# USCbiostats/bayesnetworks

Measured on NVIDIA B200. Metric: edge_proposals_scored_per_sec, higher is better.
Workload: dtype f64

## Files before the change

bayesnetworks_b200/api.py:

```python
from __future__ import annotations

import ctypes as C
from dataclasses import dataclass
from typing import Optional, Sequence

import numpy as np

from . import _lib
from ._lib import BN_RNG_REPLAY, BN_RNG_RMT, BN_RNG_WH, BnError, as_i32, check, ptr
from .network import Network

TRACE_COLUMNS = ("iter", "ChangedNode", "movetype", "globalLL", "additions", "deletions", "FN", "FP")
_RNG_KINDS = {"wh": BN_RNG_WH, "rmt": BN_RNG_RMT, "replay": BN_RNG_REPLAY,
              BN_RNG_WH: BN_RNG_WH, BN_RNG_RMT: BN_RNG_RMT, BN_RNG_REPLAY: BN_RNG_REPLAY}


@dataclass
class ChainResult:
    trace: dict
    uniforms: int
    valid_iters: int
    proposed: tuple
    reject: tuple
    n_nonpd: int
    total_edges: int
    windows: int
    alg_bytes: int
    phase_cycles: tuple
    slots_simulated: int
    final_parents: np.ndarray
    final_npar: np.ndarray
    accepted_moves: Optional[np.ndarray] = None
    edge_freq: Optional[np.ndarray] = None
    npar_freq: Optional[np.ndarray] = None
    kernel_cycles: int = 0
    mt_state: Optional[np.ndarray] = None
    state: Optional["ChainState"] = None

    def edges(self):
        return [(int(self.final_parents[c, e]), c)
                for c in range(len(self.final_npar)) for e in range(int(self.final_npar[c]))]


_STATE_SCALARS = ("iter", "valid", "total_edges_member", "additions", "deletions", "uniforms")


@dataclass
class ChainState:
    parents: np.ndarray
    npar: np.ndarray
    n_samples: Optional[int] = None
    rng: Optional[int] = None
    iter: int = 0
    valid: int = 1
    total_edges_member: int = 0
    additions: int = 0
    deletions: int = 0
    uniforms: int = 0
    wh_state: Optional[np.ndarray] = None
    mt_state: Optional[np.ndarray] = None
    score_block: Optional[np.ndarray] = None

    @property
    def P(self) -> int:
        return int(self.npar.shape[0])

    @property
    def max_par(self) -> int:
        return int(self.parents.shape[1])

    @property
    def resumed(self) -> bool:
        return self.rng is not None

    @classmethod
    def from_graph(cls, parents, npar) -> "ChainState":
        parents, npar = as_i32(parents), as_i32(npar)
        if parents.ndim != 2 or npar.shape != (parents.shape[0],):
            raise ValueError("parents must be (P, max_par) and npar (P,)")
        return cls(parents=parents.copy(), npar=npar.copy())

    @classmethod
    def from_edges(cls, edges, n_nodes: int, max_par: int) -> "ChainState":
        parents = np.full((n_nodes, max_par), -1, dtype=np.int32)
        npar = np.zeros(n_nodes, dtype=np.int32)
        for j, c in edges:
            if npar[c] >= max_par:
                raise ValueError(f"node {c} has more than max_par = {max_par} parents")
            parents[c, npar[c]] = j
            npar[c] += 1
        return cls(parents=parents, npar=npar)

    def save(self, path) -> None:
        d = {"parents": self.parents, "npar": self.npar}
        for k in _STATE_SCALARS:
            d[k] = np.int64(getattr(self, k))
        for k in ("n_samples", "rng"):
            if getattr(self, k) is not None:
                d[k] = np.int64(getattr(self, k))
        for k in ("wh_state", "mt_state", "score_block"):
            if getattr(self, k) is not None:
                d[k] = getattr(self, k)
        np.savez(path, **d)

    @classmethod
    def load(cls, path) -> "ChainState":
        with np.load(path) as z:
            kw = {k: int(z[k]) for k in _STATE_SCALARS}
            for k in ("n_samples", "rng"):
                kw[k] = int(z[k]) if k in z else None
            for k in ("wh_state", "mt_state", "score_block"):
                kw[k] = z[k].copy() if k in z else None
            return cls(parents=z["parents"].copy(), npar=z["npar"].copy(), **kw)


def _bad_arg(msg):
    return BnError(_lib.BN_ERR_BAD_ARG, msg)


def _i32_bits(a) -> np.ndarray:
    return np.ascontiguousarray((np.asarray(a).astype(np.int64) & 0xFFFFFFFF).astype(np.uint32).view(np.int32))


def set_default_stream(cuda_stream: Optional[int]) -> None:
    check(_lib.lib().bn_set_default_stream(C.c_void_p(cuda_stream or 0)))


class Context:

    def __init__(self, handle, n_samples, n_nodes, max_par):
        self._h = handle
        self.n_samples, self.n_nodes, self.max_par = n_samples, n_nodes, max_par

    @staticmethod
    def _graph_args(graph_source, graph_target, graph_node_type, n_nodes):
        src, tgt = as_i32(graph_source), as_i32(graph_target)
        if src.shape != tgt.shape:
            raise ValueError("graph_source and graph_target must have the same length")
        nt = as_i32(graph_node_type)
        if nt.shape != (n_nodes,):
            raise ValueError("graph_node_type must have one entry per column of X")
        return src, tgt, nt

    @classmethod
    def from_data(cls, X, graph_source, graph_target, graph_node_type, max_par=50, phi=1.0,
                  omega=6.9, device=0):
        Xf = np.asfortranarray(np.asarray(X, dtype=np.float64))
        n, p = Xf.shape
        src, tgt, nt = cls._graph_args(graph_source, graph_target, graph_node_type, p)
        h = C.c_void_p()
        check(_lib.lib().bn_create(ptr(Xf), n, p, ptr(src), ptr(tgt), len(src), ptr(nt), int(max_par),
                                   float(phi), float(omega), int(device), C.byref(h)))
        return cls(h, n, p, int(max_par))

    @classmethod
    def from_device(cls, data_ptr, ld, n_samples, n_nodes, graph_source, graph_target,
                    graph_node_type, max_par=50, phi=1.0, omega=6.9, device=0):
        src, tgt, nt = cls._graph_args(graph_source, graph_target, graph_node_type, n_nodes)
        h = C.c_void_p()
        check(_lib.lib().bn_create_from_device(C.c_void_p(int(data_ptr)), int(ld), int(n_samples),
                                               int(n_nodes), ptr(src), ptr(tgt), len(src), ptr(nt),
                                               int(max_par), float(phi), float(omega), int(device),
                                               C.byref(h)))
        return cls(h, int(n_samples), int(n_nodes), int(max_par))

    @classmethod
    def from_stats(cls, n_samples, mean, centered_gram, graph_source, graph_target,
                   graph_node_type, max_par=50, phi=1.0, omega=6.9, device=0):
        mean = np.ascontiguousarray(mean, dtype=np.float64)
        cg = np.ascontiguousarray(centered_gram, dtype=np.float64)
        p = mean.shape[0]
        if cg.shape != (p, p):
            raise ValueError("centered_gram must be (n_nodes, n_nodes)")
        src, tgt, nt = cls._graph_args(graph_source, graph_target, graph_node_type, p)
        h = C.c_void_p()
        check(_lib.lib().bn_create_from_stats(int(n_samples), p, ptr(mean), ptr(cg), ptr(src), ptr(tgt),
                                              len(src), ptr(nt), int(max_par), float(phi),
                                              float(omega), int(device), C.byref(h)))
        return cls(h, int(n_samples), p, int(max_par))

    @classmethod
    def from_stats_device(cls, n_samples, n_nodes, d_mean, d_centered_gram, graph_source, graph_target,
                          graph_node_type, max_par=50, phi=1.0, omega=6.9, device=0):
        src, tgt, nt = cls._graph_args(graph_source, graph_target, graph_node_type, n_nodes)
        h = C.c_void_p()
        check(_lib.lib().bn_create_from_stats_device(int(n_samples), int(n_nodes), C.c_void_p(int(d_mean)),
                                                     C.c_void_p(int(d_centered_gram)), ptr(src), ptr(tgt),
                                                     len(src), ptr(nt), int(max_par), float(phi), float(omega),
                                                     int(device), C.byref(h)))
        return cls(h, int(n_samples), int(n_nodes), int(max_par))

    def close(self):
        if self._h is not None and self._h.value:
            _lib.lib().bn_destroy(self._h)
            self._h = None

    def __enter__(self):
        return self

    def __exit__(self, *exc):
        self.close()

    def __del__(self):
        try:
            self.close()
        except Exception:
            pass

    def set_stream(self, cuda_stream: Optional[int]):
        check(_lib.lib().bn_set_stream(self._h, C.c_void_p(cuda_stream or 0)))

    @property
    def gram_ms(self) -> float:
        ms = C.c_float(0)
        check(_lib.lib().bn_get_gram_ms(self._h, C.byref(ms)))
        return float(ms.value)

    @property
    def launch_count(self) -> int:
        return int(_lib.lib().bn_get_launch_count(self._h))

    def stats(self):
        p = self.n_nodes
        sum_x, mean = np.empty(p), np.empty(p)
        sum_xx = np.empty((p, p), order="F")
        centered = np.empty((p, p))
        check(_lib.lib().bn_get_stats(self._h, ptr(sum_x), ptr(sum_xx), ptr(mean), ptr(centered)))
        return sum_x, np.ascontiguousarray(sum_xx), mean, centered

    def score_nodes(self, child, parents, n_par):
        child, n_par = as_i32(child), as_i32(n_par)
        parents = as_i32(parents)
        n = child.shape[0]
        if parents.shape != (n, self.max_par):
            raise ValueError(f"parents must be ({n}, {self.max_par})")
        out = np.empty(n)
        check(_lib.lib().bn_score_nodes(self._h, n, ptr(child), ptr(parents), ptr(n_par), ptr(out)))
        return out

    def score_all_proposals(self, parents, n_par, want_score=True, want_log_hr=True):
        parents, n_par = as_i32(parents), as_i32(n_par)
        if parents.ndim == 2:
            parents, n_par = parents[None], n_par[None]
        g, p = n_par.shape
        if parents.shape != (g, p, self.max_par) or p != self.n_nodes:
            raise ValueError("parents must be (n_graphs, n_nodes, max_par)")
        base = np.empty((g, p))
        score = np.empty((g, p, p)) if want_score else None
        hr = np.empty((g, p, p)) if want_log_hr else None
        check(_lib.lib().bn_score_all_proposals(self._h, g, ptr(parents), ptr(n_par), ptr(base),
                                                ptr(score), ptr(hr)))
        return base, score, hr

    def score_all_proposals_device(self, n_graphs, d_parents, d_npar, d_base, d_score, d_log_hr):
        ms = C.c_float(0)
        check(_lib.lib().bn_score_all_proposals_device(
            self._h, int(n_graphs), C.c_void_p(d_parents), C.c_void_p(d_npar), C.c_void_p(d_base or 0),
            C.c_void_p(d_score or 0), C.c_void_p(d_log_hr or 0), C.byref(ms)))
        return float(ms.value)

    @property
    def score_state_len(self) -> int:
        n = C.c_int64(0)
        check(_lib.lib().bn_score_state_len(self._h, C.byref(n)))
        return int(n.value)

    def _start_args(self, start, n_chains, kind, args, keep):
        p, mp = self.n_nodes, self.max_par
        if len(start) != n_chains:
            raise _bad_arg(f"start holds {len(start)} states for {n_chains} chains")
        for c, st in enumerate(start):
            if st.P != p or st.max_par != mp:
                raise _bad_arg(f"start state of chain {c} is for P={st.P}, max_par={st.max_par}; "
                               f"the context has P={p}, max_par={mp}")
            if st.resumed and (st.rng != kind or st.n_samples != self.n_samples):
                raise _bad_arg(f"start state of chain {c} continues a stream of kind {st.rng} over "
                               f"{st.n_samples} samples; this run is kind {kind} over {self.n_samples}")
        resumed = {st.resumed for st in start}
        if len(resumed) > 1:
            raise _bad_arg("start mixes fresh and resumed chains")
        par = np.ascontiguousarray(np.stack([as_i32(st.parents) for st in start]))
        npar = np.ascontiguousarray(np.stack([as_i32(st.npar) for st in start]))
        keep += [par, npar]
        args.start_parents, args.start_n_par = par.ctypes.data_as(_lib._ip), npar.ctypes.data_as(_lib._ip)
        if resumed.pop():
            sts = (_lib.ChainStateC * n_chains)()
            for c, st in enumerate(start):
                o = sts[c]
                for k in _STATE_SCALARS:
                    setattr(o, k, int(getattr(st, k)))
                if kind == BN_RNG_WH:
                    o.wh_state[:] = [int(v) for v in st.wh_state]
            keep.append(sts)
            args.state_in = C.cast(sts, C.c_void_p)
            if kind == BN_RNG_RMT:
                mt_in = np.ascontiguousarray(np.stack([_i32_bits(st.mt_state) for st in start]))
                keep.append(mt_in)
                args.mt_state_in = mt_in.ctypes.data_as(_lib._ip)
        blocks = [st.score_block is not None for st in start]
        if any(blocks):
            if not all(blocks):
                raise _bad_arg("start gives a score block for some chains only")
            sb = np.ascontiguousarray(np.stack([np.asarray(st.score_block, dtype=np.float64) for st in start]))
            if sb.shape[1] != self.score_state_len:
                raise _bad_arg(f"score block of {sb.shape[1]} doubles; this context needs {self.score_state_len}")
            keep.append(sb)
            args.score_state_in = sb.ctypes.data_as(_lib._dp)

    def run(self, n_chains=1, n_iter=1000, output=100, initial_network=2, drop=0, rng="wh",
            seeds=None, replay=None, log_moves=False, moves_capacity=None, tabulate=False,
            mt_state=None, want_mt_state=False, start=None, want_state=False):
        L = _lib.lib()
        kind = _RNG_KINDS[rng]
        p, mp = self.n_nodes, self.max_par
        cap = max(1, (n_iter + output - 1) // output)
        ints = {k: np.empty((n_chains, cap), dtype=np.int32) for k in
                ("iter", "ChangedNode", "movetype", "additions", "deletions", "FN", "FP")}
        gll = np.empty((n_chains, cap))
        n_rows = np.zeros(n_chains, dtype=np.int32)
        tr = _lib.Trace(cap, n_rows.ctypes.data_as(_lib._ip), ints["iter"].ctypes.data_as(_lib._ip),
                        ints["ChangedNode"].ctypes.data_as(_lib._ip),
                        ints["movetype"].ctypes.data_as(_lib._ip), gll.ctypes.data_as(_lib._dp),
                        ints["additions"].ctypes.data_as(_lib._ip),
                        ints["deletions"].ctypes.data_as(_lib._ip), ints["FN"].ctypes.data_as(_lib._ip),
                        ints["FP"].ctypes.data_as(_lib._ip))
        args = _lib.RunArgs()
        args.n_chains, args.rng_kind = int(n_chains), int(kind)
        sd = None
        if seeds is not None:
            sd = np.zeros((n_chains, 3), dtype=np.int32)
            s_in = np.asarray(seeds, dtype=np.int64)
            if s_in.ndim == 0:
                s_in = s_in.reshape(1, 1)
            if s_in.ndim == 1:
                s_in = s_in.reshape(n_chains, -1) if n_chains > 1 else s_in.reshape(1, -1)
            sd[:, :s_in.shape[1]] = s_in
            args.seeds = sd.ctypes.data_as(_lib._ip)
        rp = None
        if kind == BN_RNG_REPLAY:
            rp = np.ascontiguousarray(replay, dtype=np.float64)
            if rp.ndim == 1:
                rp = rp[None]
            if rp.shape[0] != n_chains:
                raise ValueError("replay must be (n_chains, replay_len)")
            args.replay = rp.ctypes.data_as(_lib._dp)
            args.replay_len = rp.shape[1]
        mt_in = mt_out = None
        if mt_state is not None:
            mt_in = _i32_bits(mt_state).reshape(n_chains, 625)
            args.mt_state_in = mt_in.ctypes.data_as(_lib._ip)
        if want_mt_state or mt_state is not None:
            mt_out = np.zeros((n_chains, 625), dtype=np.int32)
            args.mt_state_out = mt_out.ctypes.data_as(_lib._ip)
        args.initial_network, args.drop = int(initial_network), int(drop)
        args.n_iter, args.output_every, args.device_outputs = int(n_iter), int(output), 0
        moves = n_moves = None
        if log_moves:
            mc = int(moves_capacity if moves_capacity is not None else n_iter)
            moves = np.zeros((n_chains, max(mc, 1), 4), dtype=np.int32)
            n_moves = np.zeros(n_chains, dtype=np.int32)
            args.moves_capacity = moves.shape[1]
            args.moves = moves.ctypes.data_as(_lib._ip)
            args.n_moves = n_moves.ctypes.data_as(_lib._ip)
        freq = nfreq = None
        if tabulate:
            freq = np.zeros((n_chains, p, p), dtype=np.int32)
            args.edge_freq = freq.ctypes.data_as(_lib._ip)
            nfreq = np.zeros((n_chains, p, mp + 1), dtype=np.int32)
            args.npar_freq = nfreq.ctypes.data_as(_lib._ip)
        keep = []
        if start is not None:
            self._start_args(start, n_chains, kind, args, keep)
            if kind == BN_RNG_RMT and start[0].resumed and mt_out is None:
                mt_out = np.zeros((n_chains, 625), dtype=np.int32)
                args.mt_state_out = mt_out.ctypes.data_as(_lib._ip)
        st_out = sb_out = None
        if want_state:
            st_out = (_lib.ChainStateC * n_chains)()
            args.state_out = C.cast(st_out, C.c_void_p)
            sb_out = np.empty((n_chains, self.score_state_len))
            args.score_state_out = sb_out.ctypes.data_as(_lib._dp)
            if kind == BN_RNG_RMT and mt_out is None:
                mt_out = np.zeros((n_chains, 625), dtype=np.int32)
                args.mt_state_out = mt_out.ctypes.data_as(_lib._ip)
        fpar = np.empty((n_chains, p, mp), dtype=np.int32)
        fnpar = np.empty((n_chains, p), dtype=np.int32)
        stats = (_lib.ChainStats * n_chains)()
        ms = C.c_float(0)
        status = L.bn_run(self._h, C.byref(args), C.byref(tr), ptr(fpar), ptr(fnpar),
                          C.cast(stats, C.c_void_p), C.byref(ms))
        check(status)
        st = np.frombuffer(stats, dtype=_lib.CHAIN_STATS_DTYPE, count=n_chains)
        out = []
        for ch in range(n_chains):
            r = int(n_rows[ch])
            trace = {k: ints[k][ch, :r] for k in ("iter", "ChangedNode", "movetype")}
            trace["globalLL"] = gll[ch, :r]
            for k in ("additions", "deletions", "FN", "FP"):
                trace[k] = ints[k][ch, :r]
            s = st[ch]
            out.append(ChainResult(
                trace=trace, uniforms=int(s["uniforms"]), valid_iters=int(s["valid_iters"]),
                proposed=tuple(s["proposed"].tolist()), reject=tuple(s["reject"].tolist()), n_nonpd=int(s["n_nonpd"]),
                total_edges=int(s["total_edges"]), windows=int(s["windows"]), alg_bytes=int(s["alg_bytes"]),
                phase_cycles=tuple(s["phase_cycles"].tolist()),
                slots_simulated=int(s["slots_simulated"]), kernel_cycles=int(s["kernel_cycles"]),
                mt_state=None if mt_out is None else mt_out[ch],
                final_parents=fpar[ch],
                final_npar=fnpar[ch],
                accepted_moves=None if moves is None else moves[ch, :int(n_moves[ch])],
                edge_freq=None if freq is None else freq[ch],
                npar_freq=None if nfreq is None else nfreq[ch]))
            if st_out is not None:
                o = st_out[ch]
                out[-1].state = ChainState(
                    parents=fpar[ch].copy(), npar=fnpar[ch].copy(), n_samples=self.n_samples, rng=kind,
                    wh_state=np.array(o.wh_state[:], dtype=np.int32) if kind == BN_RNG_WH else None,
                    mt_state=mt_out[ch].copy() if kind == BN_RNG_RMT else None, score_block=sb_out[ch],
                    **{k: int(getattr(o, k)) for k in _STATE_SCALARS})
        return out, float(ms.value)


    def run_device(self, n_chains, n_iter, output, d_ints, d_gll, d_n_rows, initial_network=2, drop=0,
                   rng="wh", seeds=None):
        L = _lib.lib()
        cap = max(1, (n_iter + output - 1) // output)
        col = lambda k: C.cast(C.c_void_p(int(d_ints) + 4 * k * n_chains * cap), _lib._ip)
        tr = _lib.Trace(cap, C.cast(C.c_void_p(int(d_n_rows)), _lib._ip), col(0), col(1), col(2),
                        C.cast(C.c_void_p(int(d_gll)), _lib._dp), col(3), col(4), col(5), col(6))
        args = _lib.RunArgs()
        args.n_chains, args.rng_kind = int(n_chains), int(_RNG_KINDS[rng])
        sd = None
        if seeds is not None:
            sd = np.zeros((n_chains, 3), dtype=np.int32)
            s_in = np.asarray(seeds, dtype=np.int64).reshape(n_chains, -1)
            sd[:, :s_in.shape[1]] = s_in
            args.seeds = sd.ctypes.data_as(_lib._ip)
        args.initial_network, args.drop = int(initial_network), int(drop)
        args.n_iter, args.output_every, args.device_outputs = int(n_iter), int(output), 1
        stats = (_lib.ChainStats * n_chains)()
        ms = C.c_float(0)
        check(L.bn_run(self._h, C.byref(args), C.byref(tr), None, None, C.cast(stats, C.c_void_p), C.byref(ms)))
        return np.frombuffer(stats, dtype=_lib.CHAIN_STATS_DTYPE, count=n_chains).copy(), float(ms.value)


def block_colsum_device(data_ptr, ld, n_rows, n_nodes, out_ptr, device=0, stream=0):
    check(_lib.lib().bn_block_colsum_device(C.c_void_p(int(data_ptr)), int(ld), int(n_rows), int(n_nodes),
                                            C.c_void_p(int(out_ptr)), int(device), C.c_void_p(int(stream))))


def block_gram_device(data_ptr, ld, n_rows, n_nodes, mean_ptr, out_ptr, device=0, stream=0):
    ms = C.c_float(0)
    check(_lib.lib().bn_block_gram_device(C.c_void_p(int(data_ptr)), int(ld), int(n_rows), int(n_nodes),
                                          C.c_void_p(int(mean_ptr)), C.c_void_p(int(out_ptr)), int(device),
                                          C.c_void_p(int(stream)), C.byref(ms)))
    return float(ms.value)


def main_fun(X, graph_source: Sequence[int], graph_target: Sequence[int],
             graph_node_labels: Sequence[int], graph_node_type: Sequence[int], MaxPar: int = 50,
             phi: float = 1, omega: float = 6.9, InitialNetwork: int = 2, drop: int = 0,
             N: int = 1000, output: int = 10, *, rng="wh", seed=None, random_seed=None) -> dict:
    Xf = np.asfortranarray(np.asarray(X, dtype=np.float64))
    n, p = Xf.shape
    src, tgt = as_i32(graph_source), as_i32(graph_target)
    labels, nt = as_i32(graph_node_labels), as_i32(graph_node_type)
    if src.shape != tgt.shape:
        raise ValueError("graph_source and graph_target must have the same length")
    kind = _RNG_KINDS[rng]
    sd = None
    if seed is not None:
        sd = np.zeros(3, dtype=np.int32)
        s_in = np.atleast_1d(np.asarray(seed, dtype=np.int64))
        sd[:len(s_in)] = s_in
    st_in = st_out = None
    if random_seed is not None:
        rs = np.asarray(random_seed, dtype=np.int64)
        if rs.shape != (626,) or rs[0] % 100 != 3:
            raise ValueError("random_seed must be R's .Random.seed of the Mersenne-Twister (626 ints, kind %%100 == 3)")
        kind = BN_RNG_RMT
        st_in = _i32_bits(rs[1:])
        st_out = np.zeros(625, dtype=np.int32)
    elif kind == BN_RNG_RMT and seed is None:
        raise ValueError("rng='rmt' needs seed= (the value given to set.seed) or random_seed=")
    cap = max(1, (int(N) + int(output) - 1) // int(output)) if output > 0 else 1
    cols = {k: np.zeros(cap, dtype=np.float64 if k == "globalLL" else np.int32) for k in TRACE_COLUMNS}
    rows = _lib.lib().bn_main_fun(ptr(Xf), n, p, ptr(src), ptr(tgt), len(src), ptr(labels), ptr(nt),
                                  int(MaxPar), float(phi), float(omega), int(InitialNetwork),
                                  int(drop), int(N), int(output), int(kind), ptr(sd), cap,
                                  *[ptr(cols[k]) for k in TRACE_COLUMNS], ptr(st_in), ptr(st_out))
    if rows < 0:
        raise BnError(-rows, _lib.lib().bn_last_error().decode("utf-8", "replace"))
    out = {k: cols[k][:rows].copy() for k in TRACE_COLUMNS}
    if st_out is not None:
        out[".Random.seed"] = np.concatenate([[int(np.asarray(random_seed)[0])], st_out]).astype(np.int32)
    return out


def bn_mcmc(X, graph: Network, MaxPar: int = 50, phi: float = 1, omega: float = 6.9,
            InitialNetwork: int = 2, drop: int = 0, N: int = 1000, output: int = 100, *,
            rng="wh", seed=None, random_seed=None) -> dict:
    return main_fun(X=X, graph_target=graph.target, graph_source=graph.source,
                    graph_node_labels=np.arange(graph.n_nodes, dtype=np.int32),
                    graph_node_type=graph.node_type_codes(), MaxPar=MaxPar, phi=phi, omega=omega,
                    InitialNetwork=InitialNetwork, drop=drop, N=N, output=output, rng=rng, seed=seed,
                    random_seed=random_seed)
```

bayesnetworks_b200/csrc/bn_api.cu:

```cuda
#include <cuda_runtime.h>
#include <stdarg.h>
#include <stdio.h>
#include <stdlib.h>
#include <string.h>

#include <algorithm>
#include <string>
#include <vector>

#include "../../include/bn_b200.h"
#include "gram.h"
#include "kernels.h"

using namespace bn;

static thread_local char g_err[512] = "";

static int fail(int code, const char* fmt, ...) {
  va_list ap;
  va_start(ap, fmt);
  vsnprintf(g_err, sizeof(g_err), fmt, ap);
  va_end(ap);
  return code;
}

#define CU_TRY(expr)                                                                        \
  do {                                                                                      \
    cudaError_t e_ = (expr);                                                                \
    if (e_ != cudaSuccess)                                                                  \
      return fail(e_ == cudaErrorMemoryAllocation ? BN_ERR_OOM : BN_ERR_CUDA, "%s: %s (%s:%d)", \
                  #expr, cudaGetErrorString(e_), __FILE__, __LINE__);                       \
  } while (0)

static thread_local cudaStream_t g_default_stream = nullptr;

extern "C" const char* bn_last_error(void) { return g_err; }
extern "C" int bn_set_default_stream(void* s) { g_default_stream = (cudaStream_t)s; return BN_OK; }
extern "C" int bn_abi_version(void) { return BN_B200_ABI_VERSION; }
extern "C" int bn_device_count(void) {
  int n = 0;
  if (cudaGetDeviceCount(&n) != cudaSuccess) { cudaGetLastError(); return 0; }
  return n;
}

#include <mutex>
namespace {
struct PoolBlock { void* p; size_t n; int dev; bool used; };
std::mutex g_pool_mu;
std::vector<PoolBlock> g_pool;
const size_t kPoolMaxBlock = (size_t)8 << 30;

bool pool_enabled() {
  static int on = -1;
  if (on < 0) { const char* e = getenv("BN_B200_POOL"); on = (e && e[0] == '0') ? 0 : 1; }
  return on == 1;
}

cudaError_t pool_alloc(void** out, size_t n) {
  if (n == 0) n = 1;
  int dev = 0;
  cudaGetDevice(&dev);
  if (pool_enabled()) {
    std::lock_guard<std::mutex> lk(g_pool_mu);
    int best = -1;
    for (int i = 0; i < (int)g_pool.size(); i++) {
      PoolBlock& b = g_pool[i];
      if (!b.used && b.dev == dev && b.n >= n && b.n <= 2 * n + (1 << 20) &&
          (best < 0 || b.n < g_pool[best].n))
        best = i;
    }
    if (best >= 0) { g_pool[best].used = true; *out = g_pool[best].p; return cudaSuccess; }
  }
  cudaError_t e = cudaMalloc(out, n);
  if (e != cudaSuccess && pool_enabled()) {
    std::lock_guard<std::mutex> lk(g_pool_mu);
    cudaGetLastError();
    for (auto it = g_pool.begin(); it != g_pool.end();)
      if (!it->used && it->dev == dev) { cudaFree(it->p); it = g_pool.erase(it); } else ++it;
    e = cudaMalloc(out, n);
  }
  if (e == cudaSuccess && pool_enabled() && n <= kPoolMaxBlock) {
    std::lock_guard<std::mutex> lk(g_pool_mu);
    g_pool.push_back({*out, n, dev, true});
  }
  return e;
}

void pool_free(void* p) {
  if (!p) return;
  {
    std::lock_guard<std::mutex> lk(g_pool_mu);
    for (PoolBlock& b : g_pool)
      if (b.p == p) { b.used = false; return; }
  }
  cudaFree(p);
}
}

extern "C" int bn_trim_pool(void) {
  std::lock_guard<std::mutex> lk(g_pool_mu);
  for (auto it = g_pool.begin(); it != g_pool.end();)
    if (!it->used) { cudaSetDevice(it->dev); cudaFree(it->p); it = g_pool.erase(it); } else ++it;
  return BN_OK;
}

#include <chrono>
namespace {
struct StageTimer {
  bool on;
  std::chrono::steady_clock::time_point t;
  const char* fn;
  explicit StageTimer(const char* f) : fn(f) {
    static int env = -1;
    if (env < 0) { const char* e = getenv("BN_B200_TIMING"); env = (e && e[0] == '1') ? 1 : 0; }
    on = env == 1;
    if (on) t = std::chrono::steady_clock::now();
  }
  void lap(const char* what) {
    if (!on) return;
    const auto n = std::chrono::steady_clock::now();
    fprintf(stderr, "[bn timing] %s: %s %.3f ms\n", fn, what, std::chrono::duration<double, std::milli>(n - t).count());
    t = n;
  }
};
}

__global__ void colsum_from_mean_kernel(const double* __restrict__ mean, int n_samples, int P,
                                        double* __restrict__ colsum) {
  const int p = blockIdx.x * blockDim.x + threadIdx.x;
  if (p < P) colsum[p] = mean[p] * (double)n_samples;
}

struct bn_ctx {
  int device = 0;
  int n_sms = 148;
  cudaStream_t own_stream = nullptr;
  cudaStream_t stream = nullptr;
  int n_samples = 0, P = 0, max_par = 0, n_sim_edges = 0;
  double phi = 1, omega = 6.9;
  double* d_C = nullptr;
  double* d_diag = nullptr;
  double* d_mean = nullptr;
  double* d_colsum = nullptr;
  uint8_t* d_node_type = nullptr;
  uint8_t* d_sim_edge = nullptr;
  int* d_prior_par = nullptr;
  int* d_prior_npar = nullptr;
  int prior_stride = 1;
  float gram_ms = 0.f;
  int64_t launches = 0;
  std::vector<void*> owned;
};

template <typename T>
static cudaError_t dalloc(bn_ctx* c, T** p, size_t n) {
  cudaError_t e = pool_alloc((void**)p, n * sizeof(T));
  if (e == cudaSuccess && c) c->owned.push_back((void*)*p);
  return e;
}

extern "C" void bn_destroy(bn_ctx* c) {
  if (!c) return;
  cudaSetDevice(c->device);
  for (void* p : c->owned) pool_free(p);
  if (c->own_stream) cudaStreamDestroy(c->own_stream);
  delete c;
}

static int check_graph_args(int n_samples, int P, const int* src, const int* tgt, int n_edges,
                            const int* node_type, int max_par) {
  if (n_samples < 3) return fail(BN_ERR_BAD_ARG, "n_samples must be >= 3 (got %d)", n_samples);
  if (P < 2 || P > 65535) return fail(BN_ERR_BAD_ARG, "n_nodes must be in [2, 65535] (got %d)", P);
  if (max_par < 1) return fail(BN_ERR_BAD_ARG, "max_par must be >= 1 (got %d)", max_par);
  if (max_par > 64) return fail(BN_ERR_UNSUPPORTED, "max_par > 64 is not supported (got %d)", max_par);
  if (n_edges < 0 || (n_edges > 0 && (!src || !tgt))) return fail(BN_ERR_BAD_ARG, "bad edge list");
  if (!node_type) return fail(BN_ERR_BAD_ARG, "node_type is NULL");
  for (int p = 0; p < P; p++)
    if (node_type[p] < 0 || node_type[p] > 2)
      return fail(BN_ERR_BAD_ARG, "node_type[%d] = %d is not 0/1/2", p, node_type[p]);
  for (int e = 0; e < n_edges; e++)
    if (src[e] < 1 || src[e] > P || tgt[e] < 1 || tgt[e] > P)
      return fail(BN_ERR_BAD_ARG, "edge %d (%d -> %d) out of range 1..%d", e, src[e], tgt[e], P);
  return BN_OK;
}

static int ctx_begin(int n_samples, int P, const int* src, const int* tgt, int n_edges, const int* node_type,
                     int max_par, double phi, double omega, int device, bn_ctx** out) {
  if (!out) return fail(BN_ERR_BAD_ARG, "out is NULL");
  *out = nullptr;
  StageTimer tm("ctx_begin");
  int rc = check_graph_args(n_samples, P, src, tgt, n_edges, node_type, max_par);
  if (rc) return rc;
  int ndev = bn_device_count();
  if (ndev <= 0) return fail(BN_ERR_NO_DEVICE, "no CUDA device available (libbn_b200 has no CPU path)");
  if (device < 0 || device >= ndev) return fail(BN_ERR_NO_DEVICE, "device %d out of range (0..%d)", device, ndev - 1);
  CU_TRY(cudaSetDevice(device));
  bn_ctx* c = new bn_ctx();
  c->device = device;
  c->n_samples = n_samples; c->P = P; c->max_par = max_par; c->phi = phi; c->omega = omega;
  tm.lap("args+device");
  int n_sms = 0;
  if (cudaDeviceGetAttribute(&n_sms, cudaDevAttrMultiProcessorCount, device) == cudaSuccess && n_sms > 0) c->n_sms = n_sms;
  tm.lap("device attributes");
  *out = c;
  CU_TRY(cudaStreamCreateWithFlags(&c->own_stream, cudaStreamNonBlocking));
  tm.lap("stream create");
  c->stream = g_default_stream ? g_default_stream : c->own_stream;

  std::vector<int> npar(P, 0);
  for (int e = 0; e < n_edges; e++) npar[tgt[e] - 1]++;
  int stride = 1;
  for (int p = 0; p < P; p++) if (npar[p] > stride) stride = npar[p];
  c->prior_stride = stride;
  std::fill(npar.begin(), npar.end(), 0);
  std::vector<int> par((size_t)P * stride, -1);
  std::vector<uint8_t> sim((size_t)P * P, 0), types(P);
  for (int e = 0; e < n_edges; e++) {
    const int child = tgt[e] - 1, parent = src[e] - 1;
    par[(size_t)child * stride + npar[child]++] = parent;
    sim[(size_t)parent + (size_t)child * P] = 1;
    c->n_sim_edges++;
  }
  for (int p = 0; p < P; p++) types[p] = (uint8_t)node_type[p];
  tm.lap("host graph arrays");
  CU_TRY(dalloc(c, &c->d_prior_par, par.size()));
  CU_TRY(dalloc(c, &c->d_prior_npar, npar.size()));
  CU_TRY(dalloc(c, &c->d_sim_edge, sim.size()));
  CU_TRY(dalloc(c, &c->d_node_type, types.size()));
  CU_TRY(dalloc(c, &c->d_C, (size_t)P * P));
  CU_TRY(dalloc(c, &c->d_diag, (size_t)P));
  CU_TRY(dalloc(c, &c->d_mean, (size_t)P));
  CU_TRY(dalloc(c, &c->d_colsum, (size_t)P));
  tm.lap("device allocations");
  CU_TRY(cudaMemcpy(c->d_prior_par, par.data(), par.size() * sizeof(int), cudaMemcpyHostToDevice));
  CU_TRY(cudaMemcpy(c->d_prior_npar, npar.data(), npar.size() * sizeof(int), cudaMemcpyHostToDevice));
  CU_TRY(cudaMemcpy(c->d_sim_edge, sim.data(), sim.size(), cudaMemcpyHostToDevice));
  CU_TRY(cudaMemcpy(c->d_node_type, types.data(), types.size(), cudaMemcpyHostToDevice));
  tm.lap("graph upload");
  return BN_OK;
}

static int ctx_build_gram(bn_ctx* c, const double* dX, int64_t ldx, double* dXc, const GramPlan& pl,
                          const double* hX = nullptr) {
  double *d_partial = nullptr, *d_scratch = nullptr;
  int* d_flag = nullptr;
  StageTimer tm("ctx_build_gram");
  CU_TRY(pool_alloc((void**)&d_partial, (size_t)pl.workspace_bytes));
  cudaError_t e1 = pool_alloc((void**)&d_scratch, (size_t)c->P * GRAM_MEAN_MAX_CHUNKS * sizeof(double));
  cudaError_t e2 = pool_alloc((void**)&d_flag, sizeof(int));
  int rc = BN_OK;
  cudaEvent_t ev0 = nullptr, ev1 = nullptr;
  if (e1 != cudaSuccess || e2 != cudaSuccess) rc = fail(BN_ERR_OOM, "gram scratch allocation failed");
  tm.lap("workspace");
  cudaStream_t copy_stream = nullptr;
  std::vector<cudaEvent_t> arrived;
  if (!rc) {
    cudaEventCreate(&ev0); cudaEventCreate(&ev1);
    cudaEventRecord(ev0, c->stream);
    const char* msg;
    if (hX) {
      if (cudaStreamCreateWithFlags(&copy_stream, cudaStreamNonBlocking) != cudaSuccess) {
        rc = fail(BN_ERR_CUDA, "cannot create the copy stream");
      } else {
        arrived.resize(pl.n_tiles);
        for (auto& e : arrived) cudaEventCreateWithFlags(&e, cudaEventDisableTiming);
        cudaEvent_t start;
        cudaEventCreateWithFlags(&start, cudaEventDisableTiming);
        cudaEventRecord(start, c->stream);
        cudaStreamWaitEvent(copy_stream, start, 0);
        cudaEventDestroy(start);
        msg = gram_build_from_host(hX, c->n_samples, c->P, dXc, pl.ld_centered, d_partial, pl, c->d_colsum,
                                   c->d_mean, c->d_C, c->P, d_scratch, d_flag, c->stream, copy_stream,
                                   arrived.data(), &c->launches);
        if (msg) rc = fail(BN_ERR_CUDA, "gram_build_from_host: %s", msg);
      }
    } else {
      msg = gram_build(dX, ldx, c->n_samples, c->P, dXc, pl.ld_centered, d_partial, pl, c->d_colsum,
                       c->d_mean, c->d_C, c->P, d_scratch, d_flag, c->stream, &c->launches);
      if (msg) rc = fail(BN_ERR_CUDA, "gram_build: %s", msg);
    }
  }
  if (!rc) {
    launch_diag(c->d_C, c->P, c->P, c->d_diag, c->stream);
    c->launches++;
    cudaEventRecord(ev1, c->stream);
    cudaError_t e = cudaStreamSynchronize(c->stream);
    if (e == cudaSuccess) e = cudaGetLastError();
    if (e != cudaSuccess) rc = fail(BN_ERR_CUDA, "gram kernels: %s", cudaGetErrorString(e));
  }
  if (!rc) {
    cudaEventElapsedTime(&c->gram_ms, ev0, ev1);
    int flag = 0;
    cudaMemcpy(&flag, d_flag, sizeof(int), cudaMemcpyDeviceToHost);
    if (flag) rc = fail(BN_ERR_CUDA, "gram_dmma_kernel: TMA pipeline timed out (flag %d)", flag);
  }
  if (ev0) cudaEventDestroy(ev0);
  if (ev1) cudaEventDestroy(ev1);
  if (copy_stream) { cudaStreamSynchronize(copy_stream); cudaStreamDestroy(copy_stream); }
  for (auto& e : arrived) cudaEventDestroy(e);
  pool_free(d_partial); pool_free(d_scratch); pool_free(d_flag);
  tm.lap("launch + sync (incl. pending H2D)");
  return rc;
}

extern "C" int bn_create(const double* X, int n_samples, int P, const int* src, const int* tgt, int n_edges,
                         const int* node_type, int max_par, double phi, double omega, int device,
                         bn_ctx** out) {
  if (!X) return fail(BN_ERR_BAD_ARG, "X is NULL");
  int rc = ctx_begin(n_samples, P, src, tgt, n_edges, node_type, max_par, phi, omega, device, out);
  if (rc) { if (out && *out) { bn_destroy(*out); *out = nullptr; } return rc; }
  bn_ctx* c = *out;
  StageTimer tm("bn_create");
  const GramPlan pl = gram_plan(n_samples, P, c->n_sms);
  double* dXc = nullptr;
  cudaError_t e = pool_alloc((void**)&dXc, (size_t)pl.ld_centered * P * sizeof(double));
  if (e != cudaSuccess) { bn_destroy(c); *out = nullptr; return fail(BN_ERR_OOM, "cannot allocate the device copy of X"); }
  tm.lap("alloc device copy of X");
  if (!rc) rc = ctx_build_gram(c, dXc, pl.ld_centered, dXc, pl, X);
  pool_free(dXc);
  if (rc) { bn_destroy(c); *out = nullptr; }
  return rc;
}

extern "C" int bn_create_from_device(const double* dX, int64_t ld, int n_samples, int P, const int* src,
                                     const int* tgt, int n_edges, const int* node_type, int max_par,
                                     double phi, double omega, int device, bn_ctx** out) {
  if (!dX) return fail(BN_ERR_BAD_ARG, "dX is NULL");
  if (ld < n_samples) return fail(BN_ERR_BAD_ARG, "ld < n_samples");
  int rc = ctx_begin(n_samples, P, src, tgt, n_edges, node_type, max_par, phi, omega, device, out);
  if (rc) { if (out && *out) { bn_destroy(*out); *out = nullptr; } return rc; }
  bn_ctx* c = *out;
  const GramPlan pl = gram_plan(n_samples, P, c->n_sms);
  double* dXc = nullptr;
  cudaError_t e = pool_alloc((void**)&dXc, (size_t)pl.ld_centered * P * sizeof(double));
  if (e != cudaSuccess) { bn_destroy(c); *out = nullptr; return fail(BN_ERR_OOM, "cannot allocate the centred copy of X"); }
  rc = ctx_build_gram(c, dX, ld, dXc, pl);
  pool_free(dXc);
  if (rc) { bn_destroy(c); *out = nullptr; }
  return rc;
}

extern "C" int bn_create_from_stats(int n_samples, int P, const double* mean, const double* centered,
                                    const int* src, const int* tgt, int n_edges, const int* node_type,
                                    int max_par, double phi, double omega, int device, bn_ctx** out) {
  if (!mean || !centered) return fail(BN_ERR_BAD_ARG, "mean/centered_gram is NULL");
  int rc = ctx_begin(n_samples, P, src, tgt, n_edges, node_type, max_par, phi, omega, device, out);
  if (rc) { if (out && *out) { bn_destroy(*out); *out = nullptr; } return rc; }
  bn_ctx* c = *out;
  std::vector<double> colsum(P);
  for (int p = 0; p < P; p++) colsum[p] = mean[p] * (double)n_samples;
  cudaError_t e = cudaMemcpy(c->d_C, centered, (size_t)P * P * 8, cudaMemcpyHostToDevice);
  if (e == cudaSuccess) e = cudaMemcpy(c->d_mean, mean, (size_t)P * 8, cudaMemcpyHostToDevice);
  if (e == cudaSuccess) e = cudaMemcpy(c->d_colsum, colsum.data(), (size_t)P * 8, cudaMemcpyHostToDevice);
  if (e == cudaSuccess) {
    launch_diag(c->d_C, P, P, c->d_diag, c->stream);
    c->launches++;
    e = cudaStreamSynchronize(c->stream);
  }
  if (e != cudaSuccess) {
    rc = fail(BN_ERR_CUDA, "upload of sufficient statistics: %s", cudaGetErrorString(e));
    bn_destroy(c); *out = nullptr;
  }
  return rc;
}

extern "C" int bn_block_colsum_device(const double* dX, int64_t ld, int n_rows, int P, double* d_out_sum,
                                      int device, void* stream) {
  if (!dX || !d_out_sum) return fail(BN_ERR_BAD_ARG, "NULL argument");
  if (n_rows < 1 || P < 1 || ld < n_rows) return fail(BN_ERR_BAD_ARG, "bad block shape");
  int ndev = bn_device_count();
  if (ndev <= 0) return fail(BN_ERR_NO_DEVICE, "no CUDA device available (libbn_b200 has no CPU path)");
  if (device < 0 || device >= ndev) return fail(BN_ERR_NO_DEVICE, "device %d out of range", device);
  CU_TRY(cudaSetDevice(device));
  cudaStream_t st = stream ? (cudaStream_t)stream : g_default_stream;
  double *d_part = nullptr, *d_mean = nullptr;
  CU_TRY(pool_alloc((void**)&d_part, (size_t)P * GRAM_MEAN_MAX_CHUNKS * sizeof(double)));
  cudaError_t e = pool_alloc((void**)&d_mean, (size_t)P * sizeof(double));
  if (e == cudaSuccess) {
    gram_column_sums(dX, ld, n_rows, P, d_part, d_out_sum, d_mean, st);
    e = cudaStreamSynchronize(st);
    if (e == cudaSuccess) e = cudaGetLastError();
  }
  pool_free(d_part); pool_free(d_mean);
  if (e != cudaSuccess) return fail(BN_ERR_CUDA, "block column sums: %s", cudaGetErrorString(e));
  return BN_OK;
}

extern "C" int bn_block_gram_device(const double* dX, int64_t ld, int n_rows, int P, const double* d_mean,
                                    double* d_out_gram, int device, void* stream, float* ms) {
  if (!dX || !d_mean || !d_out_gram) return fail(BN_ERR_BAD_ARG, "NULL argument");
  if (n_rows < 1 || P < 2 || ld < n_rows) return fail(BN_ERR_BAD_ARG, "bad block shape");
  int ndev = bn_device_count();
  if (ndev <= 0) return fail(BN_ERR_NO_DEVICE, "no CUDA device available (libbn_b200 has no CPU path)");
  if (device < 0 || device >= ndev) return fail(BN_ERR_NO_DEVICE, "device %d out of range", device);
  CU_TRY(cudaSetDevice(device));
  cudaStream_t st = stream ? (cudaStream_t)stream : g_default_stream;
  int n_sms = 148;
  cudaDeviceGetAttribute(&n_sms, cudaDevAttrMultiProcessorCount, device);
  const GramPlan pl = gram_plan(n_rows, P, n_sms);
  double *dXc = nullptr, *d_partial = nullptr;
  int* d_flag = nullptr;
  cudaError_t e = pool_alloc((void**)&dXc, (size_t)pl.ld_centered * P * sizeof(double));
  if (e == cudaSuccess) e = pool_alloc((void**)&d_partial, (size_t)pl.workspace_bytes);
  if (e == cudaSuccess) e = pool_alloc((void**)&d_flag, sizeof(int));
  int rc = BN_OK;
  if (e != cudaSuccess) rc = fail(BN_ERR_OOM, "block gram workspace allocation failed");
  cudaEvent_t ev0 = nullptr, ev1 = nullptr;
  if (!rc) {
    cudaEventCreate(&ev0); cudaEventCreate(&ev1);
    cudaEventRecord(ev0, st);
    const char* msg = gram_build(dX, ld, n_rows, P, dXc, pl.ld_centered, d_partial, pl, nullptr,
                                 const_cast<double*>(d_mean), d_out_gram, P, nullptr, d_flag, st, nullptr, true);
    if (msg) rc = fail(BN_ERR_CUDA, "gram_build: %s", msg);
  }
  if (!rc) {
    cudaEventRecord(ev1, st);
    e = cudaStreamSynchronize(st);
    if (e == cudaSuccess) e = cudaGetLastError();
    if (e != cudaSuccess) rc = fail(BN_ERR_CUDA, "block gram kernels: %s", cudaGetErrorString(e));
  }
  if (!rc) {
    float t = 0.f;
    cudaEventElapsedTime(&t, ev0, ev1);
    if (ms) *ms = t;
    int flag = 0;
    cudaMemcpy(&flag, d_flag, sizeof(int), cudaMemcpyDeviceToHost);
    if (flag) rc = fail(BN_ERR_CUDA, "gram_dmma_kernel: TMA pipeline timed out (flag %d)", flag);
  }
  if (ev0) cudaEventDestroy(ev0);
  if (ev1) cudaEventDestroy(ev1);
  pool_free(dXc); pool_free(d_partial); pool_free(d_flag);
  return rc;
}

extern "C" int bn_create_from_stats_device(int n_samples, int P, const double* d_mean, const double* d_centered,
                                           const int* src, const int* tgt, int n_edges, const int* node_type,
                                           int max_par, double phi, double omega, int device, bn_ctx** out) {
  if (!d_mean || !d_centered) return fail(BN_ERR_BAD_ARG, "mean/centered_gram is NULL");
  int rc = ctx_begin(n_samples, P, src, tgt, n_edges, node_type, max_par, phi, omega, device, out);
  if (rc) { if (out && *out) { bn_destroy(*out); *out = nullptr; } return rc; }
  bn_ctx* c = *out;
  cudaError_t e = cudaMemcpyAsync(c->d_C, d_centered, (size_t)P * P * 8, cudaMemcpyDeviceToDevice, c->stream);
  if (e == cudaSuccess) e = cudaMemcpyAsync(c->d_mean, d_mean, (size_t)P * 8, cudaMemcpyDeviceToDevice, c->stream);
  if (e == cudaSuccess) {
    colsum_from_mean_kernel<<<(P + 127) / 128, 128, 0, c->stream>>>(c->d_mean, n_samples, P, c->d_colsum);
    launch_diag(c->d_C, P, P, c->d_diag, c->stream);
    c->launches += 2;
    e = cudaStreamSynchronize(c->stream);
    if (e == cudaSuccess) e = cudaGetLastError();
  }
  if (e != cudaSuccess) {
    rc = fail(BN_ERR_CUDA, "device sufficient statistics: %s", cudaGetErrorString(e));
    bn_destroy(c); *out = nullptr;
  }
  return rc;
}

extern "C" int bn_set_stream(bn_ctx* c, void* s) {
  if (!c) return fail(BN_ERR_BAD_ARG, "ctx is NULL");
  c->stream = s ? (cudaStream_t)s : c->own_stream;
  return BN_OK;
}

extern "C" int bn_get_gram_ms(bn_ctx* c, float* ms) {
  if (!c || !ms) return fail(BN_ERR_BAD_ARG, "NULL argument");
  *ms = c->gram_ms;
  return BN_OK;
}

extern "C" int64_t bn_get_launch_count(bn_ctx* c) { return c ? c->launches : 0; }

extern "C" int bn_get_stats(bn_ctx* c, double* sum_x, double* sum_xx, double* mean, double* centered) {
  if (!c) return fail(BN_ERR_BAD_ARG, "ctx is NULL");
  CU_TRY(cudaSetDevice(c->device));
  const int P = c->P;
  std::vector<double> C((size_t)P * P), cs(P), mu(P);
  CU_TRY(cudaMemcpy(C.data(), c->d_C, C.size() * 8, cudaMemcpyDeviceToHost));
  CU_TRY(cudaMemcpy(cs.data(), c->d_colsum, (size_t)P * 8, cudaMemcpyDeviceToHost));
  CU_TRY(cudaMemcpy(mu.data(), c->d_mean, (size_t)P * 8, cudaMemcpyDeviceToHost));
  if (sum_x) memcpy(sum_x, cs.data(), (size_t)P * 8);
  if (mean) memcpy(mean, mu.data(), (size_t)P * 8);
  if (centered) memcpy(centered, C.data(), C.size() * 8);
  if (sum_xx) {
    const double n = (double)c->n_samples;
    for (int a = 0; a < P; a++)
      for (int b = 0; b < P; b++) sum_xx[(size_t)a + (size_t)b * P] = C[(size_t)a * P + b] + n * mu[a] * mu[b];
  }
  return BN_OK;
}

extern "C" int bn_score_nodes(bn_ctx* c, int n_items, const int* child, const int* parents, const int* n_par,
                              double* out_ll) {
  if (!c || !child || !parents || !n_par || !out_ll) return fail(BN_ERR_BAD_ARG, "NULL argument");
  if (n_items <= 0) return BN_OK;
  for (int i = 0; i < n_items; i++) {
    if (child[i] < 0 || child[i] >= c->P) return fail(BN_ERR_BAD_ARG, "child[%d] out of range", i);
    if (n_par[i] < 0 || n_par[i] > c->max_par) return fail(BN_ERR_BAD_ARG, "n_par[%d] out of range", i);
    if (c->n_samples - n_par[i] - 1 <= 0) return fail(BN_ERR_BAD_ARG, "n_par[%d] leaves no degrees of freedom", i);
    for (int e = 0; e < n_par[i]; e++) {
      const int q = parents[(size_t)i * c->max_par + e];
      if (q < 0 || q >= c->P) return fail(BN_ERR_BAD_ARG, "parents[%d][%d] out of range", i, e);
    }
  }
  CU_TRY(cudaSetDevice(c->device));
  int *d_child = nullptr, *d_par = nullptr, *d_np = nullptr, *d_npd = nullptr;
  double* d_out = nullptr;
  int rc = BN_OK;
  cudaError_t e = pool_alloc((void**)&d_child, (size_t)n_items * 4);
  if (e == cudaSuccess) e = pool_alloc((void**)&d_par, (size_t)n_items * c->max_par * 4);
  if (e == cudaSuccess) e = pool_alloc((void**)&d_np, (size_t)n_items * 4);
  if (e == cudaSuccess) e = pool_alloc((void**)&d_npd, 4);
  if (e == cudaSuccess) e = pool_alloc((void**)&d_out, (size_t)n_items * 8);
  if (e == cudaSuccess) e = cudaMemcpyAsync(d_child, child, (size_t)n_items * 4, cudaMemcpyHostToDevice, c->stream);
  if (e == cudaSuccess) e = cudaMemcpyAsync(d_par, parents, (size_t)n_items * c->max_par * 4, cudaMemcpyHostToDevice, c->stream);
  if (e == cudaSuccess) e = cudaMemcpyAsync(d_np, n_par, (size_t)n_items * 4, cudaMemcpyHostToDevice, c->stream);
  if (e == cudaSuccess) e = cudaMemsetAsync(d_npd, 0, 4, c->stream);
  if (e == cudaSuccess) {
    const char* msg = launch_score_nodes(c->d_C, c->P, c->n_samples, c->max_par, n_items, d_child, d_par, d_np,
                                         d_out, d_npd, c->stream);
    c->launches++;
    if (msg) rc = fail(BN_ERR_UNSUPPORTED, "%s", msg);
  }
  if (e == cudaSuccess && !rc) e = cudaMemcpyAsync(out_ll, d_out, (size_t)n_items * 8, cudaMemcpyDeviceToHost, c->stream);
  if (e == cudaSuccess && !rc) e = cudaStreamSynchronize(c->stream);
  if (e != cudaSuccess) rc = fail(e == cudaErrorMemoryAllocation ? BN_ERR_OOM : BN_ERR_CUDA, "bn_score_nodes: %s", cudaGetErrorString(e));
  pool_free(d_child); pool_free(d_par); pool_free(d_np); pool_free(d_npd); pool_free(d_out);
  return rc;
}

static int sweep_device(bn_ctx* c, int n_graphs, const int* d_parents, const int* d_npar, double* d_base,
                        double* d_score, double* d_hr, float* kernel_ms) {
  int *d_te = nullptr, *d_ag = nullptr;
  CU_TRY(pool_alloc((void**)&d_te, (size_t)n_graphs * 4));
  cudaError_t e = pool_alloc((void**)&d_ag, (size_t)n_graphs * 4);
  if (e != cudaSuccess) { pool_free(d_te); return fail(BN_ERR_OOM, "sweep scratch"); }
  int* d_order = nullptr;
  {
    const char* so = getenv("BN_B200_SWEEP_ORDER");
    if (!(so && so[0] == '0') && (int64_t)n_graphs * c->P < (1ll << 31)) {
      e = pool_alloc((void**)&d_order, (size_t)n_graphs * c->P * 4);
      if (e != cudaSuccess) { pool_free(d_te); pool_free(d_ag); return fail(BN_ERR_OOM, "sweep scratch"); }
    }
  }
  SweepParams sp;
  sp.P = c->P; sp.max_par = c->max_par; sp.n_graphs = n_graphs; sp.n_samples = c->n_samples;
  sp.n_sim_edges = c->n_sim_edges; sp.C = c->d_C; sp.ldc = c->P; sp.diag = c->d_diag;
  sp.node_type = c->d_node_type; sp.sim_edge = c->d_sim_edge; sp.phi = c->phi; sp.omega = c->omega;
  sp.parents = d_parents; sp.n_par = d_npar; sp.te = d_te; sp.agree = d_ag; sp.order = d_order;
  sp.out_base = d_base; sp.out_score = d_score; sp.out_log_hr = d_hr;
  cudaEvent_t ev0, ev1;
  cudaEventCreate(&ev0); cudaEventCreate(&ev1);
  cudaEventRecord(ev0, c->stream);
  const char* msg = launch_sweep(sp, c->stream);
  c->launches += d_order ? 3 : 2;
  cudaEventRecord(ev1, c->stream);
  int rc = BN_OK;
  if (msg) rc = fail(BN_ERR_UNSUPPORTED, "%s", msg);
  e = cudaStreamSynchronize(c->stream);
  if (e == cudaSuccess) e = cudaGetLastError();
  if (e != cudaSuccess && !rc) rc = fail(BN_ERR_CUDA, "sweep kernel: %s", cudaGetErrorString(e));
  if (!rc && kernel_ms) cudaEventElapsedTime(kernel_ms, ev0, ev1);
  cudaEventDestroy(ev0); cudaEventDestroy(ev1);
  pool_free(d_te); pool_free(d_ag);
  if (d_order) pool_free(d_order);
  return rc;
}

extern "C" int bn_score_all_proposals_device(bn_ctx* c, int n_graphs, const int* d_parents, const int* d_npar,
                                             double* d_base, double* d_score, double* d_hr, float* kernel_ms) {
  if (!c || !d_parents || !d_npar) return fail(BN_ERR_BAD_ARG, "NULL argument");
  if (n_graphs <= 0) return fail(BN_ERR_BAD_ARG, "n_graphs <= 0");
  CU_TRY(cudaSetDevice(c->device));
  return sweep_device(c, n_graphs, d_parents, d_npar, d_base, d_score, d_hr, kernel_ms);
}

extern "C" int bn_score_all_proposals(bn_ctx* c, int n_graphs, const int* parents, const int* n_par,
                                      double* out_base, double* out_score, double* out_log_hr) {
  if (!c || !parents || !n_par) return fail(BN_ERR_BAD_ARG, "NULL argument");
  if (n_graphs <= 0) return fail(BN_ERR_BAD_ARG, "n_graphs <= 0");
  const int P = c->P, MP = c->max_par;
  for (int64_t i = 0; i < (int64_t)n_graphs * P; i++) {
    if (n_par[i] < 0 || n_par[i] > MP) return fail(BN_ERR_BAD_ARG, "n_par[%lld] out of range", (long long)i);
    for (int e = 0; e < n_par[i]; e++) {
      const int q = parents[i * MP + e];
      if (q < 0 || q >= P) return fail(BN_ERR_BAD_ARG, "parents[%lld][%d] out of range", (long long)i, e);
    }
  }
  CU_TRY(cudaSetDevice(c->device));
  const size_t npp = (size_t)n_graphs * P * P;
  int *d_par = nullptr, *d_np = nullptr;
  double *d_base = nullptr, *d_score = nullptr, *d_hr = nullptr;
  cudaError_t e = pool_alloc((void**)&d_par, (size_t)n_graphs * P * MP * 4);
  if (e == cudaSuccess) e = pool_alloc((void**)&d_np, (size_t)n_graphs * P * 4);
  if (e == cudaSuccess) e = pool_alloc((void**)&d_base, (size_t)n_graphs * P * 8);
  if (e == cudaSuccess && out_score) e = pool_alloc((void**)&d_score, npp * 8);
  if (e == cudaSuccess && out_log_hr) e = pool_alloc((void**)&d_hr, npp * 8);
  if (e == cudaSuccess) e = cudaMemcpy(d_par, parents, (size_t)n_graphs * P * MP * 4, cudaMemcpyHostToDevice);
  if (e == cudaSuccess) e = cudaMemcpy(d_np, n_par, (size_t)n_graphs * P * 4, cudaMemcpyHostToDevice);
  int rc = BN_OK;
  if (e != cudaSuccess) rc = fail(e == cudaErrorMemoryAllocation ? BN_ERR_OOM : BN_ERR_CUDA, "bn_score_all_proposals: %s", cudaGetErrorString(e));
  if (!rc) rc = sweep_device(c, n_graphs, d_par, d_np, d_base, d_score, d_hr, nullptr);
  if (!rc) {
    if (out_base) e = cudaMemcpy(out_base, d_base, (size_t)n_graphs * P * 8, cudaMemcpyDeviceToHost);
    if (e == cudaSuccess && out_score) e = cudaMemcpy(out_score, d_score, npp * 8, cudaMemcpyDeviceToHost);
    if (e == cudaSuccess && out_log_hr) e = cudaMemcpy(out_log_hr, d_hr, npp * 8, cudaMemcpyDeviceToHost);
    if (e != cudaSuccess) rc = fail(BN_ERR_CUDA, "bn_score_all_proposals D2H: %s", cudaGetErrorString(e));
  }
  pool_free(d_par); pool_free(d_np); pool_free(d_base); pool_free(d_score); pool_free(d_hr);
  return rc;
}

static uint64_t splitmix64(uint64_t& x) {
  uint64_t z = (x += 0x9E3779B97F4A7C15ull);
  z = (z ^ (z >> 30)) * 0xBF58476D1CE4E5B9ull;
  z = (z ^ (z >> 27)) * 0x94D049BB133111EBull;
  return z ^ (z >> 31);
}

static void rmt_seed_state(uint32_t seed, uint32_t* mt) {
  for (int j = 0; j < 50; j++) seed = 69069u * seed + 1u;
  for (int j = 0; j < 625; j++) {
    seed = 69069u * seed + 1u;
    if (j > 0) mt[j - 1] = seed;
  }
}

static int check_start_graphs(int nc, int P, int MP, const int* par, const int* npar) {
  std::vector<int> indeg(P), order, kids_n(P), kids_off(P + 1), kids;
  for (int ch = 0; ch < nc; ch++) {
    const int* pc = par + (size_t)ch * P * MP;
    const int* nc_ = npar + (size_t)ch * P;
    std::fill(kids_n.begin(), kids_n.end(), 0);
    for (int c = 0; c < P; c++) {
      const int k = nc_[c];
      if (k < 0 || k > MP) return fail(BN_ERR_BAD_ARG, "start graph of chain %d: node %d has %d parents (max_par = %d)", ch, c, k, MP);
      for (int e = 0; e < MP; e++) {
        const int q = pc[(size_t)c * MP + e];
        if (e >= k) {
          if (q != -1) return fail(BN_ERR_BAD_ARG, "start graph of chain %d: node %d, slot %d beyond its %d parents is not -1", ch, c, e, k);
          continue;
        }
        if (q < 0 || q >= P) return fail(BN_ERR_BAD_ARG, "start graph of chain %d: node %d has parent %d out of range", ch, c, q);
        if (q == c) return fail(BN_ERR_BAD_ARG, "start graph of chain %d: node %d is its own parent", ch, c);
        for (int f = 0; f < e; f++)
          if (pc[(size_t)c * MP + f] == q) return fail(BN_ERR_BAD_ARG, "start graph of chain %d: node %d lists parent %d twice", ch, c, q);
        kids_n[q]++;
      }
    }
    kids_off[0] = 0;
    for (int c = 0; c < P; c++) kids_off[c + 1] = kids_off[c] + kids_n[c];
    kids.assign(kids_off[P], 0);
    std::fill(kids_n.begin(), kids_n.end(), 0);
    order.clear();
    for (int c = 0; c < P; c++) {
      indeg[c] = nc_[c];
      if (!indeg[c]) order.push_back(c);
      for (int e = 0; e < nc_[c]; e++) { const int q = pc[(size_t)c * MP + e]; kids[kids_off[q] + kids_n[q]++] = c; }
    }
    for (size_t i = 0; i < order.size(); i++)
      for (int t = kids_off[order[i]]; t < kids_off[order[i] + 1]; t++)
        if (--indeg[kids[t]] == 0) order.push_back(kids[t]);
    if ((int)order.size() < P)
      for (int c = 0; c < P; c++)
        if (indeg[c] > 0) return fail(BN_ERR_BAD_ARG, "start graph of chain %d is cyclic: node %d lies on or behind a cycle", ch, c);
  }
  return BN_OK;
}

static int64_t score_state_len(int P, int MP) {
  return (int64_t)P + (MP > 8 ? (int64_t)P * fac_stride(fac_mp(MP)) : 0);
}

extern "C" int bn_score_state_len(bn_ctx* c, int64_t* n) {
  if (!c || !n) return fail(BN_ERR_BAD_ARG, "NULL argument");
  *n = score_state_len(c->P, c->max_par);
  return BN_OK;
}

struct DevBuf {
  std::vector<void*> ptrs;
  ~DevBuf() { for (void* p : ptrs) pool_free(p); }
  template <typename T>
  cudaError_t alloc(T** p, size_t n) {
    cudaError_t e = pool_alloc((void**)p, n * sizeof(T));
    if (e == cudaSuccess) ptrs.push_back((void*)*p);
    return e;
  }
};

extern "C" int bn_run(bn_ctx* c, const bn_run_args* a, bn_trace* trace, int* final_parents, int* final_n_par,
                      bn_chain_stats* stats, float* kernel_ms) {
  if (!c || !a || !trace) return fail(BN_ERR_BAD_ARG, "NULL argument");
  const int nc = a->n_chains;
  if (nc <= 0) return fail(BN_ERR_BAD_ARG, "n_chains <= 0");
  if (a->n_iter < 0 || a->output_every <= 0 || a->drop < 0) return fail(BN_ERR_BAD_ARG, "bad n_iter/output/drop");
  const int init_net = (a->initial_network == 1 || a->initial_network == 2) ? a->initial_network : 0;
  if (init_net == 0 && c->prior_stride > c->max_par)
    return fail(BN_ERR_BAD_ARG, "InitialNetwork=%d starts from the supplied graph, in which a node has %d parents (max_par=%d)",
                a->initial_network, c->prior_stride, c->max_par);
  if (a->mt_state_in && a->rng_kind != BN_RNG_RMT) return fail(BN_ERR_BAD_ARG, "mt_state_in needs rng_kind = BN_RNG_RMT");
  if (a->mt_state_out && a->rng_kind != BN_RNG_RMT) return fail(BN_ERR_BAD_ARG, "mt_state_out needs rng_kind = BN_RNG_RMT");
  if (a->rng_kind < BN_RNG_WH || a->rng_kind > BN_RNG_REPLAY) return fail(BN_ERR_BAD_ARG, "bad rng_kind");
  if (a->rng_kind == BN_RNG_REPLAY && (!a->replay || a->replay_len <= 0)) return fail(BN_ERR_BAD_ARG, "replay buffer missing");
  const int need = (a->n_iter + a->output_every - 1) / a->output_every;
  if (trace->capacity < need) return fail(BN_ERR_CAPACITY, "trace capacity %d < %d rows", trace->capacity, need);
  if (!trace->n_rows || !trace->iter || !trace->changed_node || !trace->movetype || !trace->global_ll ||
      !trace->additions || !trace->deletions || !trace->fn || !trace->fp)
    return fail(BN_ERR_BAD_ARG, "trace column pointer is NULL");
  const bool given = a->start_parents != nullptr, resume = a->state_in != nullptr;
  const bool with_state = given || a->state_out || a->score_state_out;
  if ((resume || a->score_state_in) && !given) return fail(BN_ERR_BAD_ARG, "state_in / score_state_in need start_parents");
  if (given && !a->start_n_par) return fail(BN_ERR_BAD_ARG, "start_parents needs start_n_par");
  if (resume && a->rng_kind == BN_RNG_RMT && !a->mt_state_in)
    return fail(BN_ERR_BAD_ARG, "resuming an R Mersenne-Twister stream needs mt_state_in");
  if (given) {
    const int rc = check_start_graphs(nc, c->P, c->max_par, a->start_parents, a->start_n_par);
    if (rc) return rc;
  }
  if (resume)
    for (int ch = 0; ch < nc; ch++) {
      const bn_chain_state& st = a->state_in[ch];
      if (st.iter < 0 || st.iter + a->n_iter > 0x7fffffffll)
        return fail(BN_ERR_BAD_ARG, "state_in of chain %d: iteration %lld + n_iter %d is outside 0..INT_MAX", ch,
                    (long long)st.iter, a->n_iter);
      if (st.valid != 0 && st.valid != 1) return fail(BN_ERR_BAD_ARG, "state_in of chain %d: valid = %d (0 or 1)", ch, st.valid);
    }
  CU_TRY(cudaSetDevice(c->device));

  const int64_t P = c->P, MP = c->max_par, W = (P + 31) / 32;
  const int64_t slen = score_state_len((int)P, (int)MP);
  const int64_t cap = trace->capacity > 0 ? trace->capacity : 1;
  StageTimer tm("bn_run");
  DevBuf buf;
  ChainWorkspace w;
  memset(&w, 0, sizeof(w));
  w.scratch_n = scratch_words((int)P, HELPER_WARPS + 1, 32);
  {
    const char* e = getenv("BN_B200_PIPE");
    int n_sm = 0;
    cudaDeviceGetAttribute(&n_sm, cudaDevAttrMultiProcessorCount, c->device);
    ChainParams q;
    memset(&q, 0, sizeof(q));
    q.P = (int)P; q.max_par = (int)MP; q.W = (int)W;
    const int sn = scratch_words((int)P, HELPER_WARPS, 32) > w.scratch_n ? scratch_words((int)P, HELPER_WARPS, 32) : w.scratch_n;
    w.pipeline = (e && e[0] != '0' && !with_state && MP <= 8 && 2 * nc <= n_sm && chains_can_pipeline(q, sn)) ? 1 : 0;
    if (w.pipeline) w.scratch_n = sn;
    if (w.pipeline && e && (e[0] == '3' || e[0] == '5')) w.pipeline = e[0] - '0';
  }
  const size_t dscore_n = (size_t)(nc * P * MP) * (w.pipeline ? 2 : 1);
  CU_TRY(buf.alloc(&w.par, (size_t)(nc * P * MP)));
  CU_TRY(buf.alloc(&w.born, (size_t)(nc * P * MP)));
  CU_TRY(buf.alloc(&w.npar, (size_t)(nc * P)));
  CU_TRY(buf.alloc(&w.base, (size_t)(nc * P)));
  CU_TRY(buf.alloc(&w.anc, (size_t)(nc * P * anc_stride((int)W))));
  CU_TRY(buf.alloc(&w.haspar, (size_t)(nc * W)));
  CU_TRY(buf.alloc(&w.hp_list, (size_t)(nc * P)));
  CU_TRY(buf.alloc(&w.scratch, (size_t)nc * w.scratch_n));
  CU_TRY(buf.alloc(&w.dscore, dscore_n));
  if (MP > 8) {
    CU_TRY(buf.alloc(&w.fac, (size_t)(nc * P * fac_stride(fac_mp((int)MP)))));
    CU_TRY(buf.alloc(&w.rowbuf, (size_t)nc * REPLAY_POS * row_stride(fac_mp((int)MP))));
  }
  CU_TRY(cudaMemsetAsync(w.dscore, 0xff, dscore_n * sizeof(double), c->stream));
  const bool dev_out = a->device_outputs != 0;
  if (given) {
    int *d_sp = nullptr, *d_sn = nullptr;
    CU_TRY(buf.alloc(&d_sp, (size_t)(nc * P * MP)));
    CU_TRY(buf.alloc(&d_sn, (size_t)(nc * P)));
    CU_TRY(cudaMemcpyAsync(d_sp, a->start_parents, (size_t)(nc * P * MP) * 4, cudaMemcpyHostToDevice, c->stream));
    CU_TRY(cudaMemcpyAsync(d_sn, a->start_n_par, (size_t)(nc * P) * 4, cudaMemcpyHostToDevice, c->stream));
    w.start_par = d_sp; w.start_npar = d_sn;
  }
  std::vector<ChainStart> starts;
  if (resume) {
    starts.resize(nc);
    for (int ch = 0; ch < nc; ch++) {
      const bn_chain_state& st = a->state_in[ch];
      starts[ch].iter = st.iter; starts[ch].valid = st.valid; starts[ch].te_m = st.total_edges_member;
      starts[ch].acc_add = st.additions; starts[ch].acc_del = st.deletions;
    }
    ChainStart* d_st = nullptr;
    CU_TRY(buf.alloc(&d_st, (size_t)nc));
    CU_TRY(cudaMemcpyAsync(d_st, starts.data(), sizeof(ChainStart) * nc, cudaMemcpyHostToDevice, c->stream));
    w.start = d_st;
  }
  const cudaMemcpyKind sc_in = dev_out ? cudaMemcpyDeviceToDevice : cudaMemcpyHostToDevice;
  if (a->score_state_in) {
    CU_TRY(cudaMemcpy2DAsync(w.base, P * 8, a->score_state_in, slen * 8, P * 8, nc, sc_in, c->stream));
    if (MP > 8)
      CU_TRY(cudaMemcpy2DAsync(w.fac, (slen - P) * 8, a->score_state_in + P, slen * 8, (slen - P) * 8, nc, sc_in, c->stream));
    w.scores_in = 1;
  }
  w.scores_out = a->score_state_out ? 1 : 0;
  w.with_state = with_state || a->state_in || a->score_state_in;
  if (dev_out) {
    w.t_iter = trace->iter; w.t_changed = trace->changed_node; w.t_movetype = trace->movetype;
    w.t_gll = trace->global_ll; w.t_add = trace->additions; w.t_del = trace->deletions;
    w.t_fn = trace->fn; w.t_fp = trace->fp;
  } else {
    CU_TRY(buf.alloc(&w.t_iter, (size_t)(nc * cap))); CU_TRY(buf.alloc(&w.t_changed, (size_t)(nc * cap)));
    CU_TRY(buf.alloc(&w.t_movetype, (size_t)(nc * cap))); CU_TRY(buf.alloc(&w.t_gll, (size_t)(nc * cap)));
    CU_TRY(buf.alloc(&w.t_add, (size_t)(nc * cap))); CU_TRY(buf.alloc(&w.t_del, (size_t)(nc * cap)));
    CU_TRY(buf.alloc(&w.t_fn, (size_t)(nc * cap))); CU_TRY(buf.alloc(&w.t_fp, (size_t)(nc * cap)));
  }
  const int mcap = (a->moves && a->moves_capacity > 0) ? a->moves_capacity : 0;
  if (mcap) {
    if (dev_out) w.moves = a->moves;
    else CU_TRY(buf.alloc(&w.moves, (size_t)nc * mcap * 4));
  }
  if (a->edge_freq) {
    if (dev_out) w.edge_freq = a->edge_freq;
    else CU_TRY(buf.alloc(&w.edge_freq, (size_t)(nc * P * P)));
    CU_TRY(cudaMemsetAsync(w.edge_freq, 0, (size_t)(nc * P * P) * 4, c->stream));
  }
  if (a->npar_freq) {
    if (dev_out) w.npar_freq = a->npar_freq;
    else CU_TRY(buf.alloc(&w.npar_freq, (size_t)(nc * P * (MP + 1))));
    CU_TRY(buf.alloc(&w.npar_since, (size_t)(nc * P)));
    CU_TRY(cudaMemsetAsync(w.npar_freq, 0, (size_t)(nc * P * (MP + 1)) * 4, c->stream));
  }

  ChainRngArgs ra;
  memset(&ra, 0, sizeof(ra));
  ra.kind = a->rng_kind;
  std::vector<int> seeds((size_t)3 * nc);
  if (a->seeds) {
    memcpy(seeds.data(), a->seeds, seeds.size() * sizeof(int));
  } else {
    for (int ch = 0; ch < nc; ch++) {
      if (ch == 0) { seeds[0] = 10437; seeds[1] = 13568; seeds[2] = 30524; }
      else {
        uint64_t st = 1234ull + (uint64_t)ch;
        seeds[3 * ch + 0] = 1 + (int)(splitmix64(st) % 30268ull);
        seeds[3 * ch + 1] = 1 + (int)(splitmix64(st) % 30306ull);
        seeds[3 * ch + 2] = 1 + (int)(splitmix64(st) % 30322ull);
      }
    }
  }
  if (resume && a->rng_kind == BN_RNG_WH)
    for (int ch = 0; ch < nc; ch++) memcpy(&seeds[3 * ch], a->state_in[ch].wh_state, 3 * sizeof(int));
  if (a->rng_kind == BN_RNG_WH) {
    for (int ch = 0; ch < nc; ch++) {
      const int* s = &seeds[3 * ch];
      if (s[0] < 1 || s[0] > 65535 || s[1] < 1 || s[1] > 65535 || s[2] < 1 || s[2] > 65535)
        return fail(BN_ERR_BAD_ARG, "Wichmann-Hill seeds of chain %d out of range 1..65535", ch);
    }
  }
  int* d_seeds = nullptr;
  CU_TRY(buf.alloc(&d_seeds, seeds.size()));
  CU_TRY(cudaMemcpyAsync(d_seeds, seeds.data(), seeds.size() * sizeof(int), cudaMemcpyHostToDevice, c->stream));
  ra.seeds = d_seeds;
  std::vector<uint32_t> mt;
  std::vector<int> mt_pos;
  if (a->rng_kind == BN_RNG_RMT) {
    mt.resize((size_t)624 * nc);
    mt_pos.assign(nc, 624);
    for (int ch = 0; ch < nc; ch++) {
      if (a->mt_state_in) {
        const int* st = a->mt_state_in + (size_t)625 * ch;
        mt_pos[ch] = (st[0] < 0 || st[0] > 624) ? 624 : st[0];
        for (int i = 0; i < 624; i++) mt[(size_t)624 * ch + i] = (uint32_t)st[1 + i];
      } else {
        rmt_seed_state((uint32_t)seeds[3 * ch], &mt[(size_t)624 * ch]);
      }
    }
    int* d_pos = nullptr;
    CU_TRY(buf.alloc(&ra.mt_states, mt.size() * (w.pipeline ? 2 : 1)));
    CU_TRY(buf.alloc(&d_pos, (size_t)nc));
    CU_TRY(cudaMemcpyAsync(ra.mt_states, mt.data(), mt.size() * 4, cudaMemcpyHostToDevice, c->stream));
    if (w.pipeline)
      CU_TRY(cudaMemcpyAsync(ra.mt_states + mt.size(), mt.data(), mt.size() * 4, cudaMemcpyHostToDevice, c->stream));
    CU_TRY(cudaMemcpyAsync(d_pos, mt_pos.data(), (size_t)nc * 4, cudaMemcpyHostToDevice, c->stream));
    ra.mt_pos = d_pos;
  }
  if (a->rng_kind == BN_RNG_REPLAY) {
    double* d_rep = nullptr;
    CU_TRY(buf.alloc(&d_rep, (size_t)nc * a->replay_len));
    CU_TRY(cudaMemcpyAsync(d_rep, a->replay, (size_t)nc * a->replay_len * 8, cudaMemcpyHostToDevice, c->stream));
    ra.replay = d_rep;
    ra.replay_len = a->replay_len;
  }

  ChainParams p;
  p.P = (int)P; p.max_par = (int)MP; p.W = (int)W; p.Ws = anc_stride((int)W); p.n_samples = c->n_samples;
  p.C = c->d_C; p.ldc = P; p.diag = c->d_diag; p.node_type = c->d_node_type; p.sim_edge = c->d_sim_edge;
  p.n_sim_edges = c->n_sim_edges; p.phi = c->phi; p.omega = c->omega;
  p.initial_network = init_net; p.drop = a->drop; p.n_iter = a->n_iter;
  p.output_every = a->output_every; p.trace_capacity = (int)cap; p.moves_capacity = mcap;
  p.prior_par = c->d_prior_par; p.prior_npar = c->d_prior_npar; p.prior_stride = c->prior_stride;

  ChainResult* d_res = nullptr;
  CU_TRY(buf.alloc(&d_res, (size_t)nc));
  tm.lap("workspace + seeds");
  cudaEvent_t ev0, ev1;
  cudaEventCreate(&ev0); cudaEventCreate(&ev1);
  cudaEventRecord(ev0, c->stream);
  const char* msg = launch_chains(p, w, ra, d_res, nc, c->stream);
  c->launches++;
  cudaEventRecord(ev1, c->stream);
  cudaError_t e = cudaStreamSynchronize(c->stream);
  if (e == cudaSuccess) e = cudaGetLastError();
  float ms = 0.f;
  if (e == cudaSuccess) cudaEventElapsedTime(&ms, ev0, ev1);
  cudaEventDestroy(ev0); cudaEventDestroy(ev1);
  if (msg) return fail(BN_ERR_UNSUPPORTED, "%s", msg);
  if (e != cudaSuccess) return fail(BN_ERR_CUDA, "chain kernel: %s", cudaGetErrorString(e));
  if (kernel_ms) *kernel_ms = ms;
  tm.lap("chain kernel + sync");

  std::vector<ChainResult> res(nc);
  CU_TRY(cudaMemcpy(res.data(), d_res, sizeof(ChainResult) * nc, cudaMemcpyDeviceToHost));
  int rc = BN_OK;
  if (w.pipeline && getenv("BN_B200_PIPE_STATS"))
    for (int ch = 0; ch < nc && ch < 4; ch++)
      fprintf(stderr, "[bn_b200] chain %d two-CTA: %d windows requested, %d waits for the builder, %d discarded, %d in-place rebuilds, %lld cycles\n",
              ch, res[ch].pipe[0], res[ch].pipe[1], res[ch].pipe[2], res[ch].pipe[3], (long long)res[ch].cyc_total),
      fprintf(stderr, "[bn_b200]   cycles: wait %lld, copy %lld, batch repair %lld, redo after it %lld, stale rebuilds %lld, publish %lld\n",
              res[ch].pipe_cyc[0], res[ch].pipe_cyc[1], res[ch].pipe_cyc[2], res[ch].pipe_cyc[3], res[ch].pipe_cyc[4], res[ch].pipe_cyc[5]);
  std::vector<int> nrows(nc), nmoves(nc);
  for (int ch = 0; ch < nc; ch++) {
    nrows[ch] = res[ch].n_rows;
    nmoves[ch] = res[ch].n_moves < mcap ? res[ch].n_moves : mcap;
    if (stats) {
      bn_chain_stats& s = stats[ch];
      s.uniforms = res[ch].uniforms; s.valid_iters = res[ch].valid_iters;
      for (int t = 0; t < 3; t++) { s.proposed[t] = res[ch].proposed[t]; s.reject[t] = res[ch].reject[t]; }
      s.n_nonpd = res[ch].n_nonpd; s.total_edges = res[ch].total_edges; s.status = res[ch].status;
      s.windows = res[ch].windows;
      s.alg_bytes = res[ch].alg_bytes;
      for (int t = 0; t < 12; t++) s.phase_cycles[t] = res[ch].cyc[t];
      s.slots_simulated = res[ch].slots_sim;
      s.kernel_cycles = res[ch].cyc_total;
    }
    if (res[ch].status == 95 && !rc)
      rc = fail(BN_ERR_CUDA, "chain %d: an accepted move did not fit the graph (two-CTA form: a record escaped its repair)", ch);
    if ((res[ch].status == 91 || res[ch].status == 92) && !rc)
      rc = fail(BN_ERR_CUDA, "chain %d: the two CTAs of the chain lost each other (mailbox watchdog %d)", ch, res[ch].status);
    if (res[ch].status == BN_ERR_NO_LEGAL_PROPOSAL && !rc)
      rc = fail(res[ch].status, "chain %d: no legal proposal exists (every candidate child is a source or full, or every candidate parent a sink / already a parent)", ch);
    if (a->rng_kind == BN_RNG_REPLAY && (res[ch].uniforms > a->replay_len || res[ch].status == BN_ERR_CAPACITY) && !rc)
      rc = fail(BN_ERR_CAPACITY, "chain %d consumed %lld uniforms, the replay buffer holds %lld", ch,
                (long long)res[ch].uniforms, (long long)a->replay_len);
    if (a->mt_state_out && a->rng_kind == BN_RNG_RMT) {
      int pos = mt_pos[ch];
      uint32_t* st = &mt[(size_t)624 * ch];
      rmt_advance(st, pos, res[ch].uniforms);
      int* out = a->mt_state_out + (size_t)625 * ch;
      out[0] = pos;
      for (int i = 0; i < 624; i++) out[1 + i] = (int)st[i];
    }
    if (a->state_out) {
      bn_chain_state& o = a->state_out[ch];
      memset(&o, 0, sizeof(o));
      o.iter = res[ch].end.iter; o.valid = res[ch].end.valid; o.total_edges_member = res[ch].end.te_m;
      o.additions = res[ch].end.acc_add; o.deletions = res[ch].end.acc_del;
      o.uniforms = (resume ? a->state_in[ch].uniforms : 0) + res[ch].uniforms;
      if (a->rng_kind == BN_RNG_WH) wh_advance(&seeds[3 * ch], res[ch].uniforms, o.wh_state);
    }
  }
  if (a->score_state_out) {
    const cudaMemcpyKind k = dev_out ? cudaMemcpyDeviceToDevice : cudaMemcpyDeviceToHost;
    CU_TRY(cudaMemcpy2D(a->score_state_out, slen * 8, w.base, P * 8, P * 8, nc, k));
    if (MP > 8) CU_TRY(cudaMemcpy2D(a->score_state_out + P, slen * 8, w.fac, (slen - P) * 8, (slen - P) * 8, nc, k));
  }
  const cudaMemcpyKind out_kind = dev_out ? cudaMemcpyHostToDevice : cudaMemcpyHostToHost;
  CU_TRY(cudaMemcpy(trace->n_rows, nrows.data(), (size_t)nc * 4, out_kind));
  if (a->n_moves) CU_TRY(cudaMemcpy(a->n_moves, nmoves.data(), (size_t)nc * 4, out_kind));
  if (!dev_out) {
    const size_t n = (size_t)(nc * cap);
    CU_TRY(cudaMemcpy(trace->iter, w.t_iter, n * 4, cudaMemcpyDeviceToHost));
    CU_TRY(cudaMemcpy(trace->changed_node, w.t_changed, n * 4, cudaMemcpyDeviceToHost));
    CU_TRY(cudaMemcpy(trace->movetype, w.t_movetype, n * 4, cudaMemcpyDeviceToHost));
    CU_TRY(cudaMemcpy(trace->global_ll, w.t_gll, n * 8, cudaMemcpyDeviceToHost));
    CU_TRY(cudaMemcpy(trace->additions, w.t_add, n * 4, cudaMemcpyDeviceToHost));
    CU_TRY(cudaMemcpy(trace->deletions, w.t_del, n * 4, cudaMemcpyDeviceToHost));
    CU_TRY(cudaMemcpy(trace->fn, w.t_fn, n * 4, cudaMemcpyDeviceToHost));
    CU_TRY(cudaMemcpy(trace->fp, w.t_fp, n * 4, cudaMemcpyDeviceToHost));
    if (mcap) CU_TRY(cudaMemcpy(a->moves, w.moves, (size_t)nc * mcap * 16, cudaMemcpyDeviceToHost));
    if (a->edge_freq) CU_TRY(cudaMemcpy(a->edge_freq, w.edge_freq, (size_t)(nc * P * P) * 4, cudaMemcpyDeviceToHost));
    if (a->npar_freq) CU_TRY(cudaMemcpy(a->npar_freq, w.npar_freq, (size_t)(nc * P * (MP + 1)) * 4, cudaMemcpyDeviceToHost));
  }
  const cudaMemcpyKind fin_kind = dev_out ? cudaMemcpyDeviceToDevice : cudaMemcpyDeviceToHost;
  if (final_parents) CU_TRY(cudaMemcpy(final_parents, w.par, (size_t)(nc * P * MP) * 4, fin_kind));
  if (final_n_par) CU_TRY(cudaMemcpy(final_n_par, w.npar, (size_t)(nc * P) * 4, fin_kind));
  tm.lap("results D2H");
  return rc;
}

extern "C" int bn_main_fun(const double* X, int n_samples, int n_nodes, const int* graph_source,
                           const int* graph_target, int n_edges, const int* graph_node_labels,
                           const int* graph_node_type, int MaxPar, double phi, double omega,
                           int InitialNetwork, int drop, int N, int output, int rng_kind, const int* seeds,
                           int capacity, int* iter, int* ChangedNode, int* movetype, double* globalLL,
                           int* additions, int* deletions, int* FN, int* FP, const int* mt_state_in,
                           int* mt_state_out) {
  (void)graph_node_labels;
  bn_ctx* c = nullptr;
  int rc = bn_create(X, n_samples, n_nodes, graph_source, graph_target, n_edges, graph_node_type, MaxPar, phi,
                     omega, 0, &c);
  if (rc) return -rc;
  bn_run_args a;
  memset(&a, 0, sizeof(a));
  a.n_chains = 1; a.rng_kind = rng_kind; a.seeds = seeds; a.initial_network = InitialNetwork;
  a.drop = drop; a.n_iter = N; a.output_every = output;
  a.mt_state_in = mt_state_in; a.mt_state_out = mt_state_out;
  int n_rows = 0;
  bn_trace t;
  t.capacity = capacity; t.n_rows = &n_rows; t.iter = iter; t.changed_node = ChangedNode; t.movetype = movetype;
  t.global_ll = globalLL; t.additions = additions; t.deletions = deletions; t.fn = FN; t.fp = FP;
  rc = bn_run(c, &a, &t, nullptr, nullptr, nullptr, nullptr);
  bn_destroy(c);
  return rc ? -rc : n_rows;
}
```

bayesnetworks_b200/csrc/gram.cu:

```cuda
#include <cuda.h>
#include <cuda_runtime.h>
#include <stdint.h>
#include <stdio.h>
#include <string.h>

#include <condition_variable>
#include <mutex>
#include <thread>
#include <vector>

#include "gram.h"

namespace bn {

__global__ void __launch_bounds__(256) column_sum_partial_kernel(
    const double* __restrict__ X, int64_t ldx, int n_samples, int chunks, double* __restrict__ part) {
  const int p = blockIdx.x, ch = blockIdx.y;
  const int64_t per = ((int64_t)n_samples + chunks - 1) / chunks;
  const int64_t lo = (int64_t)ch * per;
  int64_t hi = lo + per;
  if (hi > n_samples) hi = n_samples;
  const double* col = X + (int64_t)p * ldx;
  double acc = 0.0;
  for (int64_t n = lo + threadIdx.x; n < hi; n += 256) acc += col[n];
  __shared__ double sh[256];
  sh[threadIdx.x] = acc;
  __syncthreads();
  for (int o = 128; o > 0; o >>= 1) {
    if ((int)threadIdx.x < o) sh[threadIdx.x] += sh[threadIdx.x + o];
    __syncthreads();
  }
  if (threadIdx.x == 0) part[(int64_t)p * chunks + ch] = sh[0];
}

__global__ void column_mean_finish_kernel(const double* __restrict__ part, int chunks, int P,
                                          int n_samples, double* __restrict__ colsum,
                                          double* __restrict__ mean) {
  const int p = blockIdx.x * blockDim.x + threadIdx.x;
  if (p >= P) return;
  double acc = 0.0;
  for (int c = 0; c < chunks; c++) acc += part[(int64_t)p * chunks + c];
  colsum[p] = acc;
  mean[p] = acc / (double)n_samples;
}

__global__ void __launch_bounds__(256) center_kernel(const double* X, int64_t ldx, int n_samples,
                                                     const double* __restrict__ mean, double* Xc,
                                                     int64_t ldc) {
  const int p = blockIdx.y;
  const double mu = mean[p];
  const double* src = X + (int64_t)p * ldx;
  double* dst = Xc + (int64_t)p * ldc;
  for (int64_t n = (int64_t)blockIdx.x * 256 + threadIdx.x; n < ldc; n += (int64_t)gridDim.x * 256)
    dst[n] = (n < n_samples) ? (src[n] - mu) : 0.0;
}

constexpr int TILE = 128;
constexpr int BOX_K = 16;
constexpr int BOXES = 2;
constexpr int STAGE_K = BOX_K * BOXES;
constexpr int NSTAGE = 3;
constexpr int BOX_BYTES = TILE * BOX_K * 8;
constexpr int OPERAND_BYTES = BOX_BYTES * BOXES;
constexpr int STAGE_BYTES = 2 * OPERAND_BYTES;
constexpr int GRAM_CONSUMER_WARPS = 8;
constexpr int GRAM_THREADS = (GRAM_CONSUMER_WARPS + 1) * 32;
constexpr int GRAM_SMEM = NSTAGE * STAGE_BYTES + 1024  + 64 ;

__device__ __forceinline__ uint32_t smem_u32(const void* p) {
  return (uint32_t)__cvta_generic_to_shared(p);
}
__device__ __forceinline__ void mbar_init(uint64_t* bar, int count) {
  asm volatile("mbarrier.init.shared::cta.b64 [%0], %1;" ::"r"(smem_u32(bar)), "r"(count));
}
__device__ __forceinline__ void mbar_expect_tx(uint64_t* bar, uint32_t bytes) {
  asm volatile("mbarrier.arrive.expect_tx.shared::cta.b64 _, [%0], %1;" ::"r"(smem_u32(bar)), "r"(bytes)
               : "memory");
}
__device__ __forceinline__ void mbar_arrive(uint64_t* bar) {
  asm volatile("mbarrier.arrive.shared::cta.b64 _, [%0];" ::"r"(smem_u32(bar)) : "memory");
}
__device__ __forceinline__ bool mbar_wait(uint64_t* bar, uint32_t parity) {
  const uint32_t addr = smem_u32(bar);
  for (uint32_t spin = 0; spin < (1u << 24); spin++) {
    uint32_t ok;
    asm volatile(
        "{\n\t.reg .pred p;\n\t"
        "mbarrier.try_wait.parity.shared::cta.b64 p, [%1], %2;\n\t"
        "selp.u32 %0, 1, 0, p;\n\t}"
        : "=r"(ok)
        : "r"(addr), "r"(parity)
        : "memory");
    if (ok) return true;
  }
  return false;
}
__device__ __forceinline__ void tma_load_2d(void* smem_dst, const CUtensorMap* map, uint64_t* bar,
                                            int x , int y ) {
  asm volatile(
      "cp.async.bulk.tensor.2d.shared::cluster.global.mbarrier::complete_tx::bytes [%0], [%1, {%3, %4}], [%2];"
      ::"r"(smem_u32(smem_dst)), "l"(map), "r"(smem_u32(bar)), "r"(x), "r"(y)
      : "memory");
}
__device__ __forceinline__ void dmma_884(double& c0, double& c1, double a, double b) {
  asm volatile("mma.sync.aligned.m8n8k4.row.col.f64.f64.f64.f64 {%0,%1}, {%2}, {%3}, {%0,%1};"
               : "+d"(c0), "+d"(c1)
               : "d"(a), "d"(b));
}
__device__ __forceinline__ double2 lds128(uint32_t addr) {
  double2 v;
  asm volatile("ld.shared.v2.f64 {%0,%1}, [%2];" : "=d"(v.x), "=d"(v.y) : "r"(addr));
  return v;
}

__global__ void __launch_bounds__(GRAM_THREADS, 1)
gram_dmma_kernel(const __grid_constant__ CUtensorMap tmap, int n_tiles, int n_pairs,
                 int stages_total, int n_splits, double* __restrict__ partial, int* __restrict__ error_flag,
                 int tj_only) {
  extern __shared__ uint8_t smem_raw[];
  uint8_t* smem = (uint8_t*)(((uintptr_t)smem_raw + 1023) & ~(uintptr_t)1023);
  uint64_t* full = (uint64_t*)(smem + NSTAGE * STAGE_BYTES);
  uint64_t* empty = full + NSTAGE;

  const int warp = threadIdx.x >> 5, lane = threadIdx.x & 31;
  int split, ti, tj;
  if (tj_only < 0) {
    split = blockIdx.x / n_pairs;
    int pair = blockIdx.x - split * n_pairs;
    ti = 0;
    while (pair >= n_tiles - ti) { pair -= n_tiles - ti; ti++; }
    tj = ti + pair;
  } else {
    split = blockIdx.x / (tj_only + 1);
    ti = blockIdx.x - split * (tj_only + 1);
    tj = tj_only;
  }
  const int item = split * n_pairs + ti * n_tiles - (ti * (ti - 1)) / 2 + (tj - ti);
  const bool diag = (ti == tj);

  const int per = (stages_total + n_splits - 1) / n_splits;
  const int st_lo = split * per;
  int st_hi = st_lo + per;
  if (st_hi > stages_total) st_hi = stages_total;
  const int n_st = st_hi > st_lo ? st_hi - st_lo : 0;

  if (threadIdx.x == 0) {
    for (int s = 0; s < NSTAGE; s++) { mbar_init(&full[s], 1); mbar_init(&empty[s], GRAM_CONSUMER_WARPS); }
    asm volatile("fence.mbarrier_init.release.cluster;" ::: "memory");
  }
  __syncthreads();

  if (warp == GRAM_CONSUMER_WARPS) {
    if (lane == 0) {
      const uint32_t bytes = diag ? OPERAND_BYTES : STAGE_BYTES;
      for (int k = 0; k < n_st; k++) {
        const int s = k % NSTAGE;
        if (k >= NSTAGE) {
          if (!mbar_wait(&empty[s], ((k / NSTAGE) - 1) & 1)) { atomicExch(error_flag, 1); break; }
        }
        uint8_t* stage = smem + s * STAGE_BYTES;
        mbar_expect_tx(&full[s], bytes);
        const int x0 = (st_lo + k) * STAGE_K;
        for (int b = 0; b < BOXES; b++) {
          tma_load_2d(stage + b * BOX_BYTES, &tmap, &full[s], x0 + b * BOX_K, ti * TILE);
          if (!diag)
            tma_load_2d(stage + OPERAND_BYTES + b * BOX_BYTES, &tmap, &full[s], x0 + b * BOX_K, tj * TILE);
        }
      }
    }
    return;
  }

  const int wr = warp >> 2, wc = warp & 3;
  const int g = lane >> 2, t = lane & 3;
  const int rho = ((g & 1) << 2) | (g >> 1);
  uint32_t lane_off[2];
#pragma unroll
  for (int h = 0; h < 2; h++) lane_off[h] = (uint32_t)(rho * 128 + (((t + 4 * h) ^ rho) << 4));

  double acc[8][4][2];
#pragma unroll
  for (int mi = 0; mi < 8; mi++)
#pragma unroll
    for (int ni = 0; ni < 4; ni++) acc[mi][ni][0] = acc[mi][ni][1] = 0.0;

  const uint32_t smem_base = smem_u32(smem);
  bool ok = true;
  for (int k = 0; k < n_st && ok; k++) {
    const int s = k % NSTAGE;
    if (!mbar_wait(&full[s], (k / NSTAGE) & 1)) { atomicExch(error_flag, 2); ok = false; break; }
    const uint32_t a_base = smem_base + s * STAGE_BYTES + (wr * 64) * 128;
    const uint32_t b_base = smem_base + s * STAGE_BYTES + (diag ? 0 : OPERAND_BYTES) + (wc * 32) * 128;
#pragma unroll
    for (int b = 0; b < BOXES; b++) {
#pragma unroll
      for (int h = 0; h < 2; h++) {
        double2 af[8], bf[4];
#pragma unroll
        for (int mi = 0; mi < 8; mi++) af[mi] = lds128(a_base + b * BOX_BYTES + mi * 8 * 128 + lane_off[h]);
#pragma unroll
        for (int ni = 0; ni < 4; ni++) bf[ni] = lds128(b_base + b * BOX_BYTES + ni * 8 * 128 + lane_off[h]);
#pragma unroll
        for (int mi = 0; mi < 8; mi++)
#pragma unroll
          for (int ni = 0; ni < 4; ni++) {
            dmma_884(acc[mi][ni][0], acc[mi][ni][1], af[mi].x, bf[ni].x);
            dmma_884(acc[mi][ni][0], acc[mi][ni][1], af[mi].y, bf[ni].y);
          }
      }
    }
    __syncwarp();
    if (lane == 0) mbar_arrive(&empty[s]);
  }

  double* out = partial + (int64_t)item * TILE * TILE;
#pragma unroll
  for (int mi = 0; mi < 8; mi++) {
    const int r = wr * 64 + mi * 8 + rho;
#pragma unroll
    for (int ni = 0; ni < 4; ni++) {
      const int c0 = wc * 32 + ni * 8 + t;
      out[r * TILE + c0] = acc[mi][ni][0];
      out[r * TILE + c0 + 4] = acc[mi][ni][1];
    }
  }
}

__global__ void __launch_bounds__(256) gram_reduce_kernel(const double* __restrict__ partial, int n_tiles,
                                                          int n_pairs, int n_splits, int P,
                                                          double* __restrict__ C, int64_t ldc) {
  const int64_t idx = (int64_t)blockIdx.x * 256 + threadIdx.x;
  if (idx >= (int64_t)P * P) return;
  const int i = (int)(idx / P), j = (int)(idx % P);
  const int a = i < j ? i : j, b = i < j ? j : i;
  const int ta = a / TILE, tb = b / TILE;
  const int pair = ta * n_tiles - (ta * (ta - 1)) / 2 + (tb - ta);
  const int64_t off = (int64_t)(a % TILE) * TILE + (b % TILE);
  double acc = 0.0;
  for (int s = 0; s < n_splits; s++)
    acc += partial[((int64_t)s * n_pairs + pair) * TILE * TILE + off];
  C[(int64_t)i * ldc + j] = acc;
}

typedef CUresult (*encode_fn_t)(CUtensorMap*, CUtensorMapDataType, cuuint32_t, void*, const cuuint64_t*,
                                const cuuint64_t*, const cuuint32_t*, const cuuint32_t*,
                                CUtensorMapInterleave, CUtensorMapSwizzle, CUtensorMapL2promotion,
                                CUtensorMapFloatOOBfill);

static encode_fn_t get_encode_fn() {
  static encode_fn_t fn = nullptr;
  if (!fn) {
    void* p = nullptr;
    cudaDriverEntryPointQueryResult qres;
    if (cudaGetDriverEntryPoint("cuTensorMapEncodeTiled", &p, cudaEnableDefault, &qres) == cudaSuccess &&
        qres == cudaDriverEntryPointSuccess)
      fn = (encode_fn_t)p;
  }
  return fn;
}

GramPlan gram_plan(int n_samples, int P, int n_sms) {
  GramPlan pl;
  pl.n_tiles = (P + TILE - 1) / TILE;
  pl.n_pairs = pl.n_tiles * (pl.n_tiles + 1) / 2;
  pl.stages_total = (n_samples + STAGE_K - 1) / STAGE_K;
  int best = 1;
  double best_score = -1.0;
  const int max_splits_by_k = pl.stages_total / 64 > 0 ? pl.stages_total / 64 : 1;
  const int64_t ws_cap = (int64_t)3 << 30;
  for (int s = 1; s <= max_splits_by_k && s <= 4096; s++) {
    const int64_t items = (int64_t)s * pl.n_pairs;
    if (items * TILE * TILE * 8 > ws_cap && s > 1) break;
    const int64_t waves = (items + n_sms - 1) / n_sms;
    const double eff = (double)items / (double)(waves * n_sms);
    const double score = eff + 1e-3 * (double)(waves < 8 ? waves : 8);
    if (score > best_score + 1e-12) { best_score = score; best = s; }
  }
  pl.n_splits = best;
  pl.items = (int64_t)best * pl.n_pairs;
  pl.workspace_bytes = pl.items * TILE * TILE * 8;
  pl.ld_centered = ((int64_t)n_samples + 15) / 16 * 16;
  return pl;
}

void gram_column_sums(const double* dX, int64_t ldx, int n_samples, int P, double* d_scratch_part,
                      double* d_colsum, double* d_mean, cudaStream_t stream) {
  int chunks = (int)((n_samples + 65535) / 65536);
  if (chunks < 1) chunks = 1;
  if (chunks > GRAM_MEAN_MAX_CHUNKS) chunks = GRAM_MEAN_MAX_CHUNKS;
  column_sum_partial_kernel<<<dim3(P, chunks), 256, 0, stream>>>(dX, ldx, n_samples, chunks, d_scratch_part);
  column_mean_finish_kernel<<<(P + 127) / 128, 128, 0, stream>>>(d_scratch_part, chunks, P, n_samples,
                                                                  d_colsum, d_mean);
}

const char* gram_build(const double* dX, int64_t ldx, int n_samples, int P, double* dXc, int64_t ld_centered,
                       double* d_partial, const GramPlan& pl, double* d_colsum, double* d_mean,
                       double* d_C, int64_t ldc, double* d_scratch_part, int* d_error_flag,
                       cudaStream_t stream, int64_t* launches, bool mean_given) {
  if (!mean_given) {
    gram_column_sums(dX, ldx, n_samples, P, d_scratch_part, d_colsum, d_mean, stream);
    if (launches) *launches += 2;
  }
  int gx = (int)((ld_centered + 255) / 256);
  if (gx > 1024) gx = 1024;
  center_kernel<<<dim3(gx, P), 256, 0, stream>>>(dX, ldx, n_samples, d_mean, dXc, ld_centered);
  encode_fn_t enc = get_encode_fn();
  if (!enc) return "cuTensorMapEncodeTiled entry point not available";
  CUtensorMap tmap;
  cuuint64_t gdim[2] = {(cuuint64_t)n_samples, (cuuint64_t)P};
  cuuint64_t gstride[1] = {(cuuint64_t)ld_centered * 8};
  cuuint32_t box[2] = {BOX_K, TILE};
  cuuint32_t estr[2] = {1, 1};
  CUresult cr = enc(&tmap, CU_TENSOR_MAP_DATA_TYPE_FLOAT64, 2, (void*)dXc, gdim, gstride, box, estr,
                    CU_TENSOR_MAP_INTERLEAVE_NONE, CU_TENSOR_MAP_SWIZZLE_128B,
                    CU_TENSOR_MAP_L2_PROMOTION_L2_256B, CU_TENSOR_MAP_FLOAT_OOB_FILL_NONE);
  if (cr != CUDA_SUCCESS) return "cuTensorMapEncodeTiled failed";
  if (cudaFuncSetAttribute(gram_dmma_kernel, cudaFuncAttributeMaxDynamicSharedMemorySize, GRAM_SMEM) !=
      cudaSuccess)
    return "cudaFuncSetAttribute(gram_dmma_kernel) failed";
  cudaMemsetAsync(d_error_flag, 0, sizeof(int), stream);
  gram_dmma_kernel<<<(unsigned)pl.items, GRAM_THREADS, GRAM_SMEM, stream>>>(
      tmap, pl.n_tiles, pl.n_pairs, pl.stages_total, pl.n_splits, d_partial, d_error_flag, -1);
  const int64_t total = (int64_t)P * P;
  gram_reduce_kernel<<<(unsigned)((total + 255) / 256), 256, 0, stream>>>(d_partial, pl.n_tiles, pl.n_pairs,
                                                                          pl.n_splits, P, d_C, ldc);
  if (launches) *launches += 3;
  return nullptr;
}

namespace {
constexpr size_t STAGE_CHUNK = (size_t)8 << 20;
constexpr int STAGE_BUFS = 4;
constexpr int STAGE_THREADS_MAX = 16;
static int stage_threads() {
  static int n = 0;
  if (n == 0) {
    const char* e = getenv("BN_B200_STAGE_THREADS");
    if (e) {
      n = atoi(e);
    } else {
      const int hw = (int)std::thread::hardware_concurrency();
      n = hw >= 16 ? 8 : (hw >= 4 ? hw / 2 : 2);
    }
    if (n < 1) n = 1;
    if (n > STAGE_THREADS_MAX) n = STAGE_THREADS_MAX;
  }
  return n;
}

class StagePool {
 public:
  static StagePool& get() { static StagePool p; return p; }
  std::mutex use;
  bool ready() {
    if (state_ == 0) {
      state_ = -1;
      bool ok = true;
      for (int b = 0; b < STAGE_BUFS && ok; b++) {
        ok = cudaHostAlloc(&buf_[b], STAGE_CHUNK, cudaHostAllocDefault) == cudaSuccess &&
             cudaEventCreateWithFlags(&free_[b], cudaEventDisableTiming) == cudaSuccess;
      }
      if (ok) {
        for (int t = 0; t < stage_threads(); t++) workers_.emplace_back([this, t] { work(t); });
        state_ = 1;
      } else {
        cudaGetLastError();
      }
    }
    return state_ == 1;
  }
  void* buffer(int b) { return buf_[b]; }
  cudaEvent_t& event(int b) { return free_[b]; }
  void copy(void* dst, const void* src, size_t bytes) {
    std::unique_lock<std::mutex> lk(mu_);
    dst_ = (char*)dst; src_ = (const char*)src; bytes_ = bytes; pending_ = stage_threads(); gen_++;
    cv_.notify_all();
    done_.wait(lk, [this] { return pending_ == 0; });
  }

 private:
  StagePool() {}
  ~StagePool() {
    {
      std::unique_lock<std::mutex> lk(mu_);
      quit_ = true;
      cv_.notify_all();
    }
    for (auto& w : workers_) w.join();
  }
  void work(int t) {
    uint64_t seen = 0;
    for (;;) {
      std::unique_lock<std::mutex> lk(mu_);
      cv_.wait(lk, [&] { return quit_ || gen_ != seen; });
      if (quit_) return;
      seen = gen_;
      const size_t per = (bytes_ / stage_threads() + 63) & ~(size_t)63;
      const size_t lo = per * t < bytes_ ? per * t : bytes_;
      const size_t hi = lo + per < bytes_ ? lo + per : bytes_;
      char* d = dst_; const char* s = src_;
      lk.unlock();
      if (hi > lo) memcpy(d + lo, s + lo, hi - lo);
      lk.lock();
      if (--pending_ == 0) done_.notify_all();
    }
  }
  int state_ = 0;
  void* buf_[STAGE_BUFS] = {};
  cudaEvent_t free_[STAGE_BUFS] = {};
  std::vector<std::thread> workers_;
  std::mutex mu_;
  std::condition_variable cv_, done_;
  char* dst_ = nullptr; const char* src_ = nullptr;
  size_t bytes_ = 0; int pending_ = 0; uint64_t gen_ = 0; bool quit_ = false;
};

bool host_is_pageable(const void* p) {
  cudaPointerAttributes a;
  if (cudaPointerGetAttributes(&a, p) != cudaSuccess) { cudaGetLastError(); return true; }
  return a.type == cudaMemoryTypeUnregistered;
}

cudaError_t staged_block_copy(StagePool& sp, int& ring, const double* hX, int n_samples, int c0, int nc,
                              double* dst, int64_t ld_centered, cudaStream_t copy_stream) {
  const size_t col_bytes = (size_t)n_samples * 8;
  int cols_per = (int)(STAGE_CHUNK / col_bytes);
  if (cols_per < 1) return cudaErrorInvalidValue;
  for (int c = 0; c < nc; c += cols_per) {
    const int n = (nc - c < cols_per) ? nc - c : cols_per;
    const int b = ring++ % STAGE_BUFS;
    cudaError_t e = cudaEventSynchronize(sp.event(b));
    if (e != cudaSuccess) return e;
    sp.copy(sp.buffer(b), hX + (int64_t)(c0 + c) * n_samples, col_bytes * n);
    e = cudaMemcpy2DAsync(dst + (int64_t)c * ld_centered, (size_t)ld_centered * 8, sp.buffer(b), col_bytes, col_bytes,
                          (size_t)n, cudaMemcpyHostToDevice, copy_stream);
    if (e != cudaSuccess) return e;
    cudaEventRecord(sp.event(b), copy_stream);
  }
  return cudaSuccess;
}
}

const char* gram_build_from_host(const double* hX, int n_samples, int P, double* dXc, int64_t ld_centered,
                                 double* d_partial, const GramPlan& pl, double* d_colsum, double* d_mean,
                                 double* d_C, int64_t ldc, double* d_scratch_part, int* d_error_flag,
                                 cudaStream_t stream, cudaStream_t copy_stream, cudaEvent_t* block_arrived,
                                 int64_t* launches) {
  encode_fn_t enc = get_encode_fn();
  if (!enc) return "cuTensorMapEncodeTiled entry point not available";
  CUtensorMap tmap;
  cuuint64_t gdim[2] = {(cuuint64_t)n_samples, (cuuint64_t)P};
  cuuint64_t gstride[1] = {(cuuint64_t)ld_centered * 8};
  cuuint32_t box[2] = {BOX_K, TILE};
  cuuint32_t estr[2] = {1, 1};
  CUresult cr = enc(&tmap, CU_TENSOR_MAP_DATA_TYPE_FLOAT64, 2, (void*)dXc, gdim, gstride, box, estr,
                    CU_TENSOR_MAP_INTERLEAVE_NONE, CU_TENSOR_MAP_SWIZZLE_128B,
                    CU_TENSOR_MAP_L2_PROMOTION_L2_256B, CU_TENSOR_MAP_FLOAT_OOB_FILL_NONE);
  if (cr != CUDA_SUCCESS) return "cuTensorMapEncodeTiled failed";
  if (cudaFuncSetAttribute(gram_dmma_kernel, cudaFuncAttributeMaxDynamicSharedMemorySize, GRAM_SMEM) !=
      cudaSuccess)
    return "cudaFuncSetAttribute(gram_dmma_kernel) failed";
  cudaMemsetAsync(d_error_flag, 0, sizeof(int), stream);
  int chunks = (int)((n_samples + 65535) / 65536);
  if (chunks < 1) chunks = 1;
  if (chunks > GRAM_MEAN_MAX_CHUNKS) chunks = GRAM_MEAN_MAX_CHUNKS;
  int gx = (int)((ld_centered + 255) / 256);
  if (gx > 1024) gx = 1024;
  StagePool& sp = StagePool::get();
  std::unique_lock<std::mutex> stage_lock(sp.use, std::defer_lock);
  bool staged = (size_t)n_samples * P * 8 >= ((size_t)32 << 20) && (size_t)n_samples * 8 <= STAGE_CHUNK &&
                host_is_pageable(hX);
  if (staged) {
    stage_lock.lock();
    staged = sp.ready();
    if (!staged) stage_lock.unlock();
  }
  int ring = 0;
  for (int b = 0; b < pl.n_tiles; b++) {
    const int c0 = b * TILE;
    const int nc = (P - c0 < TILE) ? P - c0 : TILE;
    double* dst = dXc + (int64_t)c0 * ld_centered;
    const double* src = hX + (int64_t)c0 * n_samples;
    cudaError_t e;
    if (staged)
      e = staged_block_copy(sp, ring, hX, n_samples, c0, nc, dst, ld_centered, copy_stream);
    else if (ld_centered == n_samples)
      e = cudaMemcpyAsync(dst, src, (size_t)n_samples * nc * 8, cudaMemcpyHostToDevice, copy_stream);
    else
      e = cudaMemcpy2DAsync(dst, (size_t)ld_centered * 8, src, (size_t)n_samples * 8, (size_t)n_samples * 8,
                            (size_t)nc, cudaMemcpyHostToDevice, copy_stream);
    if (e != cudaSuccess) return "H2D copy of a column block failed";
    cudaEventRecord(block_arrived[b], copy_stream);
    cudaStreamWaitEvent(stream, block_arrived[b], 0);
    column_sum_partial_kernel<<<dim3(nc, chunks), 256, 0, stream>>>(dst, ld_centered, n_samples, chunks,
                                                                     d_scratch_part + (int64_t)c0 * chunks);
    column_mean_finish_kernel<<<(nc + 127) / 128, 128, 0, stream>>>(d_scratch_part + (int64_t)c0 * chunks, chunks,
                                                                     nc, n_samples, d_colsum + c0, d_mean + c0);
    center_kernel<<<dim3(gx, nc), 256, 0, stream>>>(dst, ld_centered, n_samples, d_mean + c0, dst, ld_centered);
    gram_dmma_kernel<<<(unsigned)(pl.n_splits * (b + 1)), GRAM_THREADS, GRAM_SMEM, stream>>>(
        tmap, pl.n_tiles, pl.n_pairs, pl.stages_total, pl.n_splits, d_partial, d_error_flag, b);
    if (launches) *launches += 4;
  }
  const int64_t total = (int64_t)P * P;
  gram_reduce_kernel<<<(unsigned)((total + 255) / 256), 256, 0, stream>>>(d_partial, pl.n_tiles, pl.n_pairs,
                                                                          pl.n_splits, P, d_C, ldc);
  if (launches) *launches += 1;
  return nullptr;
}

}
```

bayesnetworks_b200/csrc/gram.h:

```cpp
#pragma once
#include <cuda_runtime.h>
#include <stdint.h>

namespace bn {

constexpr int GRAM_MEAN_MAX_CHUNKS = 64;

struct GramPlan {
  int n_tiles;
  int n_pairs;
  int stages_total;
  int n_splits;
  int64_t items;
  int64_t workspace_bytes;
  int64_t ld_centered;
};

GramPlan gram_plan(int n_samples, int P, int n_sms);

void gram_column_sums(const double* dX, int64_t ldx, int n_samples, int P, double* d_scratch_part,
                      double* d_colsum, double* d_mean, cudaStream_t stream);

const char* gram_build(const double* dX, int64_t ldx, int n_samples, int P, double* dXc,
                       int64_t ld_centered, double* d_partial, const GramPlan& pl, double* d_colsum,
                       double* d_mean, double* d_C, int64_t ldc, double* d_scratch_part,
                       int* d_error_flag, cudaStream_t stream, int64_t* launches, bool mean_given = false);

const char* gram_build_from_host(const double* hX, int n_samples, int P, double* dXc, int64_t ld_centered,
                                 double* d_partial, const GramPlan& pl, double* d_colsum, double* d_mean,
                                 double* d_C, int64_t ldc, double* d_scratch_part, int* d_error_flag,
                                 cudaStream_t stream, cudaStream_t copy_stream, cudaEvent_t* block_arrived,
                                 int64_t* launches);

}
```

Baseline: 123.7 million.

## Defer gram sync, pin-stage graph and result transfers, vectorise centering

Context creation now queues the graph upload and Gram build asynchronously on the stream, recording an event and deferring synchronisation and scratch frees until results are needed. Host staging buffers are pinned and pooled, with graph arrays packed into a single transfer and chain results gathered into one pinned block copied asynchronously and then unpacked. The centering kernel handles two doubles per thread through double2 loads, and the Python side converts stats columns in bulk rather than per chain. This targets host-side sync and many-small-memcpy overhead, at the cost of more complex lifetime and error handling around pending work.

```diff
diff --git a/bayesnetworks_b200/api.py b/bayesnetworks_b200/api.py
--- a/bayesnetworks_b200/api.py
+++ b/bayesnetworks_b200/api.py
@@ -391,20 +391,20 @@
                           C.cast(stats, C.c_void_p), C.byref(ms))
         check(status)
         st = np.frombuffer(stats, dtype=_lib.CHAIN_STATS_DTYPE, count=n_chains)
+        col = {k: st[k].tolist() for k in ("uniforms", "valid_iters", "proposed", "reject", "n_nonpd", "total_edges",
+                                            "windows", "alg_bytes", "phase_cycles", "slots_simulated", "kernel_cycles")}
         out = []
-        for ch in range(n_chains):
-            r = int(n_rows[ch])
+        for ch, r in enumerate(n_rows.tolist()):
             trace = {k: ints[k][ch, :r] for k in ("iter", "ChangedNode", "movetype")}
             trace["globalLL"] = gll[ch, :r]
             for k in ("additions", "deletions", "FN", "FP"):
                 trace[k] = ints[k][ch, :r]
-            s = st[ch]
             out.append(ChainResult(
-                trace=trace, uniforms=int(s["uniforms"]), valid_iters=int(s["valid_iters"]),
-                proposed=tuple(s["proposed"].tolist()), reject=tuple(s["reject"].tolist()), n_nonpd=int(s["n_nonpd"]),
-                total_edges=int(s["total_edges"]), windows=int(s["windows"]), alg_bytes=int(s["alg_bytes"]),
-                phase_cycles=tuple(s["phase_cycles"].tolist()),
-                slots_simulated=int(s["slots_simulated"]), kernel_cycles=int(s["kernel_cycles"]),
+                trace=trace, uniforms=col["uniforms"][ch], valid_iters=col["valid_iters"][ch],
+                proposed=tuple(col["proposed"][ch]), reject=tuple(col["reject"][ch]), n_nonpd=col["n_nonpd"][ch],
+                total_edges=col["total_edges"][ch], windows=col["windows"][ch], alg_bytes=col["alg_bytes"][ch],
+                phase_cycles=tuple(col["phase_cycles"][ch]),
+                slots_simulated=col["slots_simulated"][ch], kernel_cycles=col["kernel_cycles"][ch],
                 mt_state=None if mt_out is None else mt_out[ch],
                 final_parents=fpar[ch],
                 final_npar=fnpar[ch],
diff --git a/bayesnetworks_b200/csrc/bn_api.cu b/bayesnetworks_b200/csrc/bn_api.cu
--- a/bayesnetworks_b200/csrc/bn_api.cu
+++ b/bayesnetworks_b200/csrc/bn_api.cu
@@ -45,7 +45,7 @@
 
 #include <mutex>
 namespace {
-struct PoolBlock { void* p; size_t n; int dev; bool used; };
+struct PoolBlock { void* p; size_t n; int dev; bool host; bool used; };
 std::mutex g_pool_mu;
 std::vector<PoolBlock> g_pool;
 const size_t kPoolMaxBlock = (size_t)8 << 30;
@@ -56,32 +56,35 @@
   return on == 1;
 }
 
-cudaError_t pool_alloc(void** out, size_t n) {
+void release_block(const PoolBlock& b) { if (b.host) cudaFreeHost(b.p); else cudaFree(b.p); }
+
+cudaError_t pool_alloc(void** out, size_t n, bool host = false) {
   if (n == 0) n = 1;
   int dev = 0;
-  cudaGetDevice(&dev);
+  if (!host) cudaGetDevice(&dev);
   if (pool_enabled()) {
     std::lock_guard<std::mutex> lk(g_pool_mu);
     int best = -1;
     for (int i = 0; i < (int)g_pool.size(); i++) {
       PoolBlock& b = g_pool[i];
-      if (!b.used && b.dev == dev && b.n >= n && b.n <= 2 * n + (1 << 20) &&
+      if (!b.used && b.host == host && b.dev == dev && b.n >= n && b.n <= 2 * n + (1 << 20) &&
           (best < 0 || b.n < g_pool[best].n))
         best = i;
     }
     if (best >= 0) { g_pool[best].used = true; *out = g_pool[best].p; return cudaSuccess; }
   }
-  cudaError_t e = cudaMalloc(out, n);
+  auto raw = [&] { return host ? cudaHostAlloc(out, n, cudaHostAllocDefault) : cudaMalloc(out, n); };
+  cudaError_t e = raw();
   if (e != cudaSuccess && pool_enabled()) {
     std::lock_guard<std::mutex> lk(g_pool_mu);
     cudaGetLastError();
     for (auto it = g_pool.begin(); it != g_pool.end();)
-      if (!it->used && it->dev == dev) { cudaFree(it->p); it = g_pool.erase(it); } else ++it;
-    e = cudaMalloc(out, n);
-  }
-  if (e == cudaSuccess && pool_enabled() && n <= kPoolMaxBlock) {
+      if (!it->used && it->host == host && it->dev == dev) { release_block(*it); it = g_pool.erase(it); } else ++it;
+    e = raw();
+  }
+  if (e == cudaSuccess && ((pool_enabled() && n <= kPoolMaxBlock) || host)) {
     std::lock_guard<std::mutex> lk(g_pool_mu);
-    g_pool.push_back({*out, n, dev, true});
+    g_pool.push_back({*out, n, dev, host, true});
   }
   return e;
 }
@@ -90,8 +93,13 @@
   if (!p) return;
   {
     std::lock_guard<std::mutex> lk(g_pool_mu);
-    for (PoolBlock& b : g_pool)
-      if (b.p == p) { b.used = false; return; }
+    for (auto it = g_pool.begin(); it != g_pool.end(); ++it)
+      if (it->p == p) {
+        if (pool_enabled()) { it->used = false; return; }
+        release_block(*it);
+        g_pool.erase(it);
+        return;
+      }
   }
   cudaFree(p);
 }
@@ -100,9 +108,17 @@
 extern "C" int bn_trim_pool(void) {
   std::lock_guard<std::mutex> lk(g_pool_mu);
   for (auto it = g_pool.begin(); it != g_pool.end();)
-    if (!it->used) { cudaSetDevice(it->dev); cudaFree(it->p); it = g_pool.erase(it); } else ++it;
+    if (!it->used) { if (!it->host) cudaSetDevice(it->dev); release_block(*it); it = g_pool.erase(it); } else ++it;
   return BN_OK;
 }
+
+struct Staging {
+  char* p = nullptr;
+  size_t n = 0;
+  size_t take(size_t bytes) { const size_t o = n; n += (bytes + 255) & ~(size_t)255; return o; }
+  cudaError_t alloc() { return pool_alloc((void**)&p, n, true); }
+  template <typename T> T* at(size_t off) const { return (T*)(p + off); }
+};
 
 #include <chrono>
 namespace {
@@ -150,6 +166,11 @@
   float gram_ms = 0.f;
   int64_t launches = 0;
   std::vector<void*> owned;
+  bool pending = false;
+  cudaEvent_t gram_ev0 = nullptr, built = nullptr;
+  int* h_flag = nullptr;
+  std::vector<void*> in_flight;
+  std::string error;
 };
 
 template <typename T>
@@ -159,9 +180,40 @@
   return e;
 }
 
+static void ctx_wait(bn_ctx* c) {
+  if (c->pending) {
+    c->pending = false;
+    cudaError_t e = cudaEventSynchronize(c->built);
+    if (e != cudaSuccess) {
+      c->error = std::string("gram kernels: ") + cudaGetErrorString(e);
+    } else {
+      if (c->gram_ev0) cudaEventElapsedTime(&c->gram_ms, c->gram_ev0, c->built);
+      if (c->h_flag && *c->h_flag) {
+        char m[96];
+        snprintf(m, sizeof(m), "gram_dmma_kernel: TMA pipeline timed out (flag %d)", *c->h_flag);
+        c->error = m;
+      }
+    }
+  }
+  for (void* p : c->in_flight) pool_free(p);
+  c->in_flight.clear();
+  pool_free(c->h_flag);
+  c->h_flag = nullptr;
+}
+
+static int ctx_settle(bn_ctx* c) {
+  ctx_wait(c);
+  if (!c->error.empty()) return fail(BN_ERR_CUDA, "%s", c->error.c_str());
+  return BN_OK;
+}
+
 extern "C" void bn_destroy(bn_ctx* c) {
   if (!c) return;
   cudaSetDevice(c->device);
+  cudaStreamSynchronize(c->stream);
+  ctx_wait(c);
+  if (c->gram_ev0) cudaEventDestroy(c->gram_ev0);
+  if (c->built) cudaEventDestroy(c->built);
   for (void* p : c->owned) pool_free(p);
   if (c->own_stream) cudaStreamDestroy(c->own_stream);
   delete c;
@@ -203,18 +255,30 @@
   if (cudaDeviceGetAttribute(&n_sms, cudaDevAttrMultiProcessorCount, device) == cudaSuccess && n_sms > 0) c->n_sms = n_sms;
   tm.lap("device attributes");
   *out = c;
-  CU_TRY(cudaStreamCreateWithFlags(&c->own_stream, cudaStreamNonBlocking));
-  tm.lap("stream create");
+  if (!g_default_stream) CU_TRY(cudaStreamCreateWithFlags(&c->own_stream, cudaStreamNonBlocking));
   c->stream = g_default_stream ? g_default_stream : c->own_stream;
-
-  std::vector<int> npar(P, 0);
-  for (int e = 0; e < n_edges; e++) npar[tgt[e] - 1]++;
+  CU_TRY(cudaEventCreate(&c->built));
+  CU_TRY(cudaEventRecord(c->built, cudaStreamLegacy));
+  CU_TRY(cudaStreamWaitEvent(c->stream, c->built, 0));
+  tm.lap("stream + events");
+
+  std::vector<int> indeg(P, 0);
+  for (int e = 0; e < n_edges; e++) indeg[tgt[e] - 1]++;
   int stride = 1;
-  for (int p = 0; p < P; p++) if (npar[p] > stride) stride = npar[p];
+  for (int p = 0; p < P; p++) if (indeg[p] > stride) stride = indeg[p];
   c->prior_stride = stride;
-  std::fill(npar.begin(), npar.end(), 0);
-  std::vector<int> par((size_t)P * stride, -1);
-  std::vector<uint8_t> sim((size_t)P * P, 0), types(P);
+  Staging st;
+  const size_t o_par = st.take((size_t)P * stride * 4), o_npar = st.take((size_t)P * 4);
+  const size_t o_sim = st.take((size_t)P * P), o_types = st.take((size_t)P);
+  CU_TRY(st.alloc());
+  c->in_flight.push_back(st.p);
+  int* par = st.at<int>(o_par);
+  int* npar = st.at<int>(o_npar);
+  uint8_t* sim = st.at<uint8_t>(o_sim);
+  uint8_t* types = st.at<uint8_t>(o_types);
+  std::fill(par, par + (size_t)P * stride, -1);
+  std::fill(npar, npar + P, 0);
+  memset(sim, 0, (size_t)P * P);
   for (int e = 0; e < n_edges; e++) {
     const int child = tgt[e] - 1, parent = src[e] - 1;
     par[(size_t)child * stride + npar[child]++] = parent;
@@ -223,20 +287,25 @@
   }
   for (int p = 0; p < P; p++) types[p] = (uint8_t)node_type[p];
   tm.lap("host graph arrays");
-  CU_TRY(dalloc(c, &c->d_prior_par, par.size()));
-  CU_TRY(dalloc(c, &c->d_prior_npar, npar.size()));
-  CU_TRY(dalloc(c, &c->d_sim_edge, sim.size()));
-  CU_TRY(dalloc(c, &c->d_node_type, types.size()));
+  char* d_graph = nullptr;
+  CU_TRY(dalloc(c, &d_graph, st.n));
+  c->d_prior_par = (int*)(d_graph + o_par);
+  c->d_prior_npar = (int*)(d_graph + o_npar);
+  c->d_sim_edge = (uint8_t*)(d_graph + o_sim);
+  c->d_node_type = (uint8_t*)(d_graph + o_types);
   CU_TRY(dalloc(c, &c->d_C, (size_t)P * P));
   CU_TRY(dalloc(c, &c->d_diag, (size_t)P));
   CU_TRY(dalloc(c, &c->d_mean, (size_t)P));
   CU_TRY(dalloc(c, &c->d_colsum, (size_t)P));
   tm.lap("device allocations");
-  CU_TRY(cudaMemcpy(c->d_prior_par, par.data(), par.size() * sizeof(int), cudaMemcpyHostToDevice));
-  CU_TRY(cudaMemcpy(c->d_prior_npar, npar.data(), npar.size() * sizeof(int), cudaMemcpyHostToDevice));
-  CU_TRY(cudaMemcpy(c->d_sim_edge, sim.data(), sim.size(), cudaMemcpyHostToDevice));
-  CU_TRY(cudaMemcpy(c->d_node_type, types.data(), types.size(), cudaMemcpyHostToDevice));
-  tm.lap("graph upload");
+  CU_TRY(cudaMemcpyAsync(d_graph, st.p, st.n, cudaMemcpyHostToDevice, c->stream));
+  tm.lap("graph upload (queued)");
+  return BN_OK;
+}
+
+static int ctx_queued(bn_ctx* c) {
+  CU_TRY(cudaEventRecord(c->built, c->stream));
+  c->pending = true;
   return BN_OK;
 }
 
@@ -245,18 +314,25 @@
   double *d_partial = nullptr, *d_scratch = nullptr;
   int* d_flag = nullptr;
   StageTimer tm("ctx_build_gram");
+  c->in_flight.push_back(dXc);
   CU_TRY(pool_alloc((void**)&d_partial, (size_t)pl.workspace_bytes));
+  c->in_flight.push_back(d_partial);
   cudaError_t e1 = pool_alloc((void**)&d_scratch, (size_t)c->P * GRAM_MEAN_MAX_CHUNKS * sizeof(double));
+  if (e1 == cudaSuccess) c->in_flight.push_back(d_scratch);
   cudaError_t e2 = pool_alloc((void**)&d_flag, sizeof(int));
+  if (e2 == cudaSuccess) c->in_flight.push_back(d_flag);
+  cudaError_t e3 = pool_alloc((void**)&c->h_flag, sizeof(int), true);
   int rc = BN_OK;
-  cudaEvent_t ev0 = nullptr, ev1 = nullptr;
-  if (e1 != cudaSuccess || e2 != cudaSuccess) rc = fail(BN_ERR_OOM, "gram scratch allocation failed");
+  if (e1 != cudaSuccess || e2 != cudaSuccess || e3 != cudaSuccess) rc = fail(BN_ERR_OOM, "gram scratch allocation failed");
   tm.lap("workspace");
   cudaStream_t copy_stream = nullptr;
+  cudaEvent_t x_read = nullptr;
   std::vector<cudaEvent_t> arrived;
+  if (!rc && (cudaEventCreate(&c->gram_ev0) != cudaSuccess ||
+              cudaEventCreateWithFlags(&x_read, cudaEventDisableTiming) != cudaSuccess))
+    rc = fail(BN_ERR_CUDA, "cannot create the gram events");
   if (!rc) {
-    cudaEventCreate(&ev0); cudaEventCreate(&ev1);
-    cudaEventRecord(ev0, c->stream);
+    cudaEventRecord(c->gram_ev0, c->stream);
     const char* msg;
     if (hX) {
       if (cudaStreamCreateWithFlags(&copy_stream, cudaStreamNonBlocking) != cudaSuccess) {
@@ -273,33 +349,31 @@
                                    c->d_mean, c->d_C, c->P, d_scratch, d_flag, c->stream, copy_stream,
                                    arrived.data(), &c->launches);
         if (msg) rc = fail(BN_ERR_CUDA, "gram_build_from_host: %s", msg);
+        cudaEventRecord(x_read, copy_stream);
       }
     } else {
       msg = gram_build(dX, ldx, c->n_samples, c->P, dXc, pl.ld_centered, d_partial, pl, c->d_colsum,
-                       c->d_mean, c->d_C, c->P, d_scratch, d_flag, c->stream, &c->launches);
+                       c->d_mean, c->d_C, c->P, d_scratch, d_flag, c->stream, &c->launches, false, x_read);
       if (msg) rc = fail(BN_ERR_CUDA, "gram_build: %s", msg);
     }
   }
   if (!rc) {
     launch_diag(c->d_C, c->P, c->P, c->d_diag, c->stream);
     c->launches++;
-    cudaEventRecord(ev1, c->stream);
-    cudaError_t e = cudaStreamSynchronize(c->stream);
-    if (e == cudaSuccess) e = cudaGetLastError();
+    const char* inj = getenv("BN_B200_INJECT_GRAM_FLAG");
+    if (inj && atoi(inj)) {
+      *c->h_flag = atoi(inj);
+      cudaMemcpyAsync(d_flag, c->h_flag, sizeof(int), cudaMemcpyHostToDevice, c->stream);
+    }
+    cudaMemcpyAsync(c->h_flag, d_flag, sizeof(int), cudaMemcpyDeviceToHost, c->stream);
+    cudaError_t e = cudaGetLastError();
     if (e != cudaSuccess) rc = fail(BN_ERR_CUDA, "gram kernels: %s", cudaGetErrorString(e));
   }
-  if (!rc) {
-    cudaEventElapsedTime(&c->gram_ms, ev0, ev1);
-    int flag = 0;
-    cudaMemcpy(&flag, d_flag, sizeof(int), cudaMemcpyDeviceToHost);
-    if (flag) rc = fail(BN_ERR_CUDA, "gram_dmma_kernel: TMA pipeline timed out (flag %d)", flag);
-  }
-  if (ev0) cudaEventDestroy(ev0);
-  if (ev1) cudaEventDestroy(ev1);
+  if (!rc) rc = ctx_queued(c);
+  if (x_read) { cudaEventSynchronize(x_read); cudaEventDestroy(x_read); }
   if (copy_stream) { cudaStreamSynchronize(copy_stream); cudaStreamDestroy(copy_stream); }
   for (auto& e : arrived) cudaEventDestroy(e);
-  pool_free(d_partial); pool_free(d_scratch); pool_free(d_flag);
-  tm.lap("launch + sync (incl. pending H2D)");
+  tm.lap("queued, X read (incl. pending H2D)");
   return rc;
 }
 
@@ -316,8 +390,7 @@
   cudaError_t e = pool_alloc((void**)&dXc, (size_t)pl.ld_centered * P * sizeof(double));
   if (e != cudaSuccess) { bn_destroy(c); *out = nullptr; return fail(BN_ERR_OOM, "cannot allocate the device copy of X"); }
   tm.lap("alloc device copy of X");
-  if (!rc) rc = ctx_build_gram(c, dXc, pl.ld_centered, dXc, pl, X);
-  pool_free(dXc);
+  rc = ctx_build_gram(c, dXc, pl.ld_centered, dXc, pl, X);
   if (rc) { bn_destroy(c); *out = nullptr; }
   return rc;
 }
@@ -335,7 +408,6 @@
   cudaError_t e = pool_alloc((void**)&dXc, (size_t)pl.ld_centered * P * sizeof(double));
   if (e != cudaSuccess) { bn_destroy(c); *out = nullptr; return fail(BN_ERR_OOM, "cannot allocate the centred copy of X"); }
   rc = ctx_build_gram(c, dX, ld, dXc, pl);
-  pool_free(dXc);
   if (rc) { bn_destroy(c); *out = nullptr; }
   return rc;
 }
@@ -360,6 +432,8 @@
   if (e != cudaSuccess) {
     rc = fail(BN_ERR_CUDA, "upload of sufficient statistics: %s", cudaGetErrorString(e));
     bn_destroy(c); *out = nullptr;
+  } else {
+    ctx_wait(c);
   }
   return rc;
 }
@@ -452,18 +526,27 @@
   if (e != cudaSuccess) {
     rc = fail(BN_ERR_CUDA, "device sufficient statistics: %s", cudaGetErrorString(e));
     bn_destroy(c); *out = nullptr;
+  } else {
+    ctx_wait(c);
   }
   return rc;
 }
 
 extern "C" int bn_set_stream(bn_ctx* c, void* s) {
   if (!c) return fail(BN_ERR_BAD_ARG, "ctx is NULL");
-  c->stream = s ? (cudaStream_t)s : c->own_stream;
+  CU_TRY(cudaSetDevice(c->device));
+  if (!s && !c->own_stream) CU_TRY(cudaStreamCreateWithFlags(&c->own_stream, cudaStreamNonBlocking));
+  cudaStream_t next = s ? (cudaStream_t)s : c->own_stream;
+  if (c->pending) CU_TRY(cudaStreamWaitEvent(next, c->built, 0));
+  c->stream = next;
   return BN_OK;
 }
 
 extern "C" int bn_get_gram_ms(bn_ctx* c, float* ms) {
   if (!c || !ms) return fail(BN_ERR_BAD_ARG, "NULL argument");
+  CU_TRY(cudaSetDevice(c->device));
+  const int rc = ctx_settle(c);
+  if (rc) return rc;
   *ms = c->gram_ms;
   return BN_OK;
 }
@@ -473,6 +556,8 @@
 extern "C" int bn_get_stats(bn_ctx* c, double* sum_x, double* sum_xx, double* mean, double* centered) {
   if (!c) return fail(BN_ERR_BAD_ARG, "ctx is NULL");
   CU_TRY(cudaSetDevice(c->device));
+  int rc = ctx_settle(c);
+  if (rc) return rc;
   const int P = c->P;
   std::vector<double> C((size_t)P * P), cs(P), mu(P);
   CU_TRY(cudaMemcpy(C.data(), c->d_C, C.size() * 8, cudaMemcpyDeviceToHost));
@@ -503,9 +588,10 @@
     }
   }
   CU_TRY(cudaSetDevice(c->device));
+  int rc = ctx_settle(c);
+  if (rc) return rc;
   int *d_child = nullptr, *d_par = nullptr, *d_np = nullptr, *d_npd = nullptr;
   double* d_out = nullptr;
-  int rc = BN_OK;
   cudaError_t e = pool_alloc((void**)&d_child, (size_t)n_items * 4);
   if (e == cudaSuccess) e = pool_alloc((void**)&d_par, (size_t)n_items * c->max_par * 4);
   if (e == cudaSuccess) e = pool_alloc((void**)&d_np, (size_t)n_items * 4);
@@ -530,6 +616,8 @@
 
 static int sweep_device(bn_ctx* c, int n_graphs, const int* d_parents, const int* d_npar, double* d_base,
                         double* d_score, double* d_hr, float* kernel_ms) {
+  const int rs = ctx_settle(c);
+  if (rs) return rs;
   int *d_te = nullptr, *d_ag = nullptr;
   CU_TRY(pool_alloc((void**)&d_te, (size_t)n_graphs * 4));
   cudaError_t e = pool_alloc((void**)&d_ag, (size_t)n_graphs * 4);
@@ -730,95 +818,9 @@
   const int64_t P = c->P, MP = c->max_par, W = (P + 31) / 32;
   const int64_t slen = score_state_len((int)P, (int)MP);
   const int64_t cap = trace->capacity > 0 ? trace->capacity : 1;
+  const bool dev_out = a->device_outputs != 0;
+  const int mcap = (a->moves && a->moves_capacity > 0) ? a->moves_capacity : 0;
   StageTimer tm("bn_run");
-  DevBuf buf;
-  ChainWorkspace w;
-  memset(&w, 0, sizeof(w));
-  w.scratch_n = scratch_words((int)P, HELPER_WARPS + 1, 32);
-  {
-    const char* e = getenv("BN_B200_PIPE");
-    int n_sm = 0;
-    cudaDeviceGetAttribute(&n_sm, cudaDevAttrMultiProcessorCount, c->device);
-    ChainParams q;
-    memset(&q, 0, sizeof(q));
-    q.P = (int)P; q.max_par = (int)MP; q.W = (int)W;
-    const int sn = scratch_words((int)P, HELPER_WARPS, 32) > w.scratch_n ? scratch_words((int)P, HELPER_WARPS, 32) : w.scratch_n;
-    w.pipeline = (e && e[0] != '0' && !with_state && MP <= 8 && 2 * nc <= n_sm && chains_can_pipeline(q, sn)) ? 1 : 0;
-    if (w.pipeline) w.scratch_n = sn;
-    if (w.pipeline && e && (e[0] == '3' || e[0] == '5')) w.pipeline = e[0] - '0';
-  }
-  const size_t dscore_n = (size_t)(nc * P * MP) * (w.pipeline ? 2 : 1);
-  CU_TRY(buf.alloc(&w.par, (size_t)(nc * P * MP)));
-  CU_TRY(buf.alloc(&w.born, (size_t)(nc * P * MP)));
-  CU_TRY(buf.alloc(&w.npar, (size_t)(nc * P)));
-  CU_TRY(buf.alloc(&w.base, (size_t)(nc * P)));
-  CU_TRY(buf.alloc(&w.anc, (size_t)(nc * P * anc_stride((int)W))));
-  CU_TRY(buf.alloc(&w.haspar, (size_t)(nc * W)));
-  CU_TRY(buf.alloc(&w.hp_list, (size_t)(nc * P)));
-  CU_TRY(buf.alloc(&w.scratch, (size_t)nc * w.scratch_n));
-  CU_TRY(buf.alloc(&w.dscore, dscore_n));
-  if (MP > 8) {
-    CU_TRY(buf.alloc(&w.fac, (size_t)(nc * P * fac_stride(fac_mp((int)MP)))));
-    CU_TRY(buf.alloc(&w.rowbuf, (size_t)nc * REPLAY_POS * row_stride(fac_mp((int)MP))));
-  }
-  CU_TRY(cudaMemsetAsync(w.dscore, 0xff, dscore_n * sizeof(double), c->stream));
-  const bool dev_out = a->device_outputs != 0;
-  if (given) {
-    int *d_sp = nullptr, *d_sn = nullptr;
-    CU_TRY(buf.alloc(&d_sp, (size_t)(nc * P * MP)));
-    CU_TRY(buf.alloc(&d_sn, (size_t)(nc * P)));
-    CU_TRY(cudaMemcpyAsync(d_sp, a->start_parents, (size_t)(nc * P * MP) * 4, cudaMemcpyHostToDevice, c->stream));
-    CU_TRY(cudaMemcpyAsync(d_sn, a->start_n_par, (size_t)(nc * P) * 4, cudaMemcpyHostToDevice, c->stream));
-    w.start_par = d_sp; w.start_npar = d_sn;
-  }
-  std::vector<ChainStart> starts;
-  if (resume) {
-    starts.resize(nc);
-    for (int ch = 0; ch < nc; ch++) {
-      const bn_chain_state& st = a->state_in[ch];
-      starts[ch].iter = st.iter; starts[ch].valid = st.valid; starts[ch].te_m = st.total_edges_member;
-      starts[ch].acc_add = st.additions; starts[ch].acc_del = st.deletions;
-    }
-    ChainStart* d_st = nullptr;
-    CU_TRY(buf.alloc(&d_st, (size_t)nc));
-    CU_TRY(cudaMemcpyAsync(d_st, starts.data(), sizeof(ChainStart) * nc, cudaMemcpyHostToDevice, c->stream));
-    w.start = d_st;
-  }
-  const cudaMemcpyKind sc_in = dev_out ? cudaMemcpyDeviceToDevice : cudaMemcpyHostToDevice;
-  if (a->score_state_in) {
-    CU_TRY(cudaMemcpy2DAsync(w.base, P * 8, a->score_state_in, slen * 8, P * 8, nc, sc_in, c->stream));
-    if (MP > 8)
-      CU_TRY(cudaMemcpy2DAsync(w.fac, (slen - P) * 8, a->score_state_in + P, slen * 8, (slen - P) * 8, nc, sc_in, c->stream));
-    w.scores_in = 1;
-  }
-  w.scores_out = a->score_state_out ? 1 : 0;
-  w.with_state = with_state || a->state_in || a->score_state_in;
-  if (dev_out) {
-    w.t_iter = trace->iter; w.t_changed = trace->changed_node; w.t_movetype = trace->movetype;
-    w.t_gll = trace->global_ll; w.t_add = trace->additions; w.t_del = trace->deletions;
-    w.t_fn = trace->fn; w.t_fp = trace->fp;
-  } else {
-    CU_TRY(buf.alloc(&w.t_iter, (size_t)(nc * cap))); CU_TRY(buf.alloc(&w.t_changed, (size_t)(nc * cap)));
-    CU_TRY(buf.alloc(&w.t_movetype, (size_t)(nc * cap))); CU_TRY(buf.alloc(&w.t_gll, (size_t)(nc * cap)));
-    CU_TRY(buf.alloc(&w.t_add, (size_t)(nc * cap))); CU_TRY(buf.alloc(&w.t_del, (size_t)(nc * cap)));
-    CU_TRY(buf.alloc(&w.t_fn, (size_t)(nc * cap))); CU_TRY(buf.alloc(&w.t_fp, (size_t)(nc * cap)));
-  }
-  const int mcap = (a->moves && a->moves_capacity > 0) ? a->moves_capacity : 0;
-  if (mcap) {
-    if (dev_out) w.moves = a->moves;
-    else CU_TRY(buf.alloc(&w.moves, (size_t)nc * mcap * 4));
-  }
-  if (a->edge_freq) {
-    if (dev_out) w.edge_freq = a->edge_freq;
-    else CU_TRY(buf.alloc(&w.edge_freq, (size_t)(nc * P * P)));
-    CU_TRY(cudaMemsetAsync(w.edge_freq, 0, (size_t)(nc * P * P) * 4, c->stream));
-  }
-  if (a->npar_freq) {
-    if (dev_out) w.npar_freq = a->npar_freq;
-    else CU_TRY(buf.alloc(&w.npar_freq, (size_t)(nc * P * (MP + 1))));
-    CU_TRY(buf.alloc(&w.npar_since, (size_t)(nc * P)));
-    CU_TRY(cudaMemsetAsync(w.npar_freq, 0, (size_t)(nc * P * (MP + 1)) * 4, c->stream));
-  }
 
   ChainRngArgs ra;
   memset(&ra, 0, sizeof(ra));
@@ -846,13 +848,10 @@
         return fail(BN_ERR_BAD_ARG, "Wichmann-Hill seeds of chain %d out of range 1..65535", ch);
     }
   }
-  int* d_seeds = nullptr;
-  CU_TRY(buf.alloc(&d_seeds, seeds.size()));
-  CU_TRY(cudaMemcpyAsync(d_seeds, seeds.data(), seeds.size() * sizeof(int), cudaMemcpyHostToDevice, c->stream));
-  ra.seeds = d_seeds;
   std::vector<uint32_t> mt;
   std::vector<int> mt_pos;
-  if (a->rng_kind == BN_RNG_RMT) {
+  const bool rmt = a->rng_kind == BN_RNG_RMT, replay = a->rng_kind == BN_RNG_REPLAY;
+  if (rmt) {
     mt.resize((size_t)624 * nc);
     mt_pos.assign(nc, 624);
     for (int ch = 0; ch < nc; ch++) {
@@ -864,19 +863,153 @@
         rmt_seed_state((uint32_t)seeds[3 * ch], &mt[(size_t)624 * ch]);
       }
     }
+  }
+
+  DevBuf buf;
+  Staging up, dn;
+  const bool sc_host = a->score_state_in && !dev_out;
+  const size_t u_seeds = up.take(seeds.size() * 4);
+  const size_t u_sp = given ? up.take((size_t)(nc * P * MP) * 4) : 0, u_sn = given ? up.take((size_t)(nc * P) * 4) : 0;
+  const size_t u_st = resume ? up.take(sizeof(ChainStart) * nc) : 0;
+  const size_t u_mt = rmt ? up.take(mt.size() * 4) : 0, u_pos = rmt ? up.take((size_t)nc * 4) : 0;
+  const size_t u_rep = replay ? up.take((size_t)nc * a->replay_len * 8) : 0;
+  const size_t u_sc = sc_host ? up.take((size_t)(nc * slen) * 8) : 0;
+  const size_t n = (size_t)(nc * cap);
+  const size_t o_res = dn.take(sizeof(ChainResult) * nc);
+  const size_t tr_bytes[8] = {n * 4, n * 4, n * 4, n * 8, n * 4, n * 4, n * 4, n * 4};
+  size_t o_tr[8] = {}, o_mv = 0, o_ef = 0, o_nf = 0, o_fp = 0, o_fn = 0, o_sc = 0;
+  if (!dev_out) {
+    for (int k = 0; k < 8; k++) o_tr[k] = dn.take(tr_bytes[k]);
+    if (mcap) o_mv = dn.take((size_t)nc * mcap * 16);
+    if (a->edge_freq) o_ef = dn.take((size_t)(nc * P * P) * 4);
+    if (a->npar_freq) o_nf = dn.take((size_t)(nc * P * (MP + 1)) * 4);
+    if (final_parents) o_fp = dn.take((size_t)(nc * P * MP) * 4);
+    if (final_n_par) o_fn = dn.take((size_t)(nc * P) * 4);
+    if (a->score_state_out) o_sc = dn.take((size_t)(nc * slen) * 8);
+  }
+  CU_TRY(up.alloc());
+  buf.ptrs.push_back(up.p);
+  CU_TRY(dn.alloc());
+  buf.ptrs.push_back(dn.p);
+  struct Drain { cudaStream_t s; ~Drain() { cudaStreamSynchronize(s); } } drain{c->stream};
+  memcpy(up.at<int>(u_seeds), seeds.data(), seeds.size() * 4);
+  if (given) {
+    memcpy(up.at<int>(u_sp), a->start_parents, (size_t)(nc * P * MP) * 4);
+    memcpy(up.at<int>(u_sn), a->start_n_par, (size_t)(nc * P) * 4);
+  }
+  if (resume)
+    for (int ch = 0; ch < nc; ch++) {
+      const bn_chain_state& st = a->state_in[ch];
+      ChainStart& s = up.at<ChainStart>(u_st)[ch];
+      memset(&s, 0, sizeof(s));
+      s.iter = st.iter; s.valid = st.valid; s.te_m = st.total_edges_member;
+      s.acc_add = st.additions; s.acc_del = st.deletions;
+    }
+  if (rmt) {
+    memcpy(up.at<uint32_t>(u_mt), mt.data(), mt.size() * 4);
+    memcpy(up.at<int>(u_pos), mt_pos.data(), (size_t)nc * 4);
+  }
+  if (replay) memcpy(up.at<double>(u_rep), a->replay, (size_t)nc * a->replay_len * 8);
+  if (sc_host) memcpy(up.at<double>(u_sc), a->score_state_in, (size_t)(nc * slen) * 8);
+  tm.lap("host inputs");
+
+  ChainWorkspace w;
+  memset(&w, 0, sizeof(w));
+  w.scratch_n = scratch_words((int)P, HELPER_WARPS + 1, 32);
+  {
+    const char* e = getenv("BN_B200_PIPE");
+    int n_sm = 0;
+    cudaDeviceGetAttribute(&n_sm, cudaDevAttrMultiProcessorCount, c->device);
+    ChainParams q;
+    memset(&q, 0, sizeof(q));
+    q.P = (int)P; q.max_par = (int)MP; q.W = (int)W;
+    const int sn = scratch_words((int)P, HELPER_WARPS, 32) > w.scratch_n ? scratch_words((int)P, HELPER_WARPS, 32) : w.scratch_n;
+    w.pipeline = (e && e[0] != '0' && !with_state && MP <= 8 && 2 * nc <= n_sm && chains_can_pipeline(q, sn)) ? 1 : 0;
+    if (w.pipeline) w.scratch_n = sn;
+    if (w.pipeline && e && (e[0] == '3' || e[0] == '5')) w.pipeline = e[0] - '0';
+  }
+  const size_t dscore_n = (size_t)(nc * P * MP) * (w.pipeline ? 2 : 1);
+  CU_TRY(buf.alloc(&w.par, (size_t)(nc * P * MP)));
+  CU_TRY(buf.alloc(&w.born, (size_t)(nc * P * MP)));
+  CU_TRY(buf.alloc(&w.npar, (size_t)(nc * P)));
+  CU_TRY(buf.alloc(&w.base, (size_t)(nc * P)));
+  CU_TRY(buf.alloc(&w.anc, (size_t)(nc * P * anc_stride((int)W))));
+  CU_TRY(buf.alloc(&w.haspar, (size_t)(nc * W)));
+  CU_TRY(buf.alloc(&w.hp_list, (size_t)(nc * P)));
+  CU_TRY(buf.alloc(&w.scratch, (size_t)nc * w.scratch_n));
+  CU_TRY(buf.alloc(&w.dscore, dscore_n));
+  if (MP > 8) {
+    CU_TRY(buf.alloc(&w.fac, (size_t)(nc * P * fac_stride(fac_mp((int)MP)))));
+    CU_TRY(buf.alloc(&w.rowbuf, (size_t)nc * REPLAY_POS * row_stride(fac_mp((int)MP))));
+  }
+  CU_TRY(cudaMemsetAsync(w.dscore, 0xff, dscore_n * sizeof(double), c->stream));
+  if (given) {
+    int *d_sp = nullptr, *d_sn = nullptr;
+    CU_TRY(buf.alloc(&d_sp, (size_t)(nc * P * MP)));
+    CU_TRY(buf.alloc(&d_sn, (size_t)(nc * P)));
+    CU_TRY(cudaMemcpyAsync(d_sp, up.p + u_sp, (size_t)(nc * P * MP) * 4, cudaMemcpyHostToDevice, c->stream));
+    CU_TRY(cudaMemcpyAsync(d_sn, up.p + u_sn, (size_t)(nc * P) * 4, cudaMemcpyHostToDevice, c->stream));
+    w.start_par = d_sp; w.start_npar = d_sn;
+  }
+  if (resume) {
+    ChainStart* d_st = nullptr;
+    CU_TRY(buf.alloc(&d_st, (size_t)nc));
+    CU_TRY(cudaMemcpyAsync(d_st, up.p + u_st, sizeof(ChainStart) * nc, cudaMemcpyHostToDevice, c->stream));
+    w.start = d_st;
+  }
+  if (a->score_state_in) {
+    const double* src = sc_host ? up.at<double>(u_sc) : a->score_state_in;
+    const cudaMemcpyKind k = sc_host ? cudaMemcpyHostToDevice : cudaMemcpyDeviceToDevice;
+    CU_TRY(cudaMemcpy2DAsync(w.base, P * 8, src, slen * 8, P * 8, nc, k, c->stream));
+    if (MP > 8)
+      CU_TRY(cudaMemcpy2DAsync(w.fac, (slen - P) * 8, src + P, slen * 8, (slen - P) * 8, nc, k, c->stream));
+    w.scores_in = 1;
+  }
+  w.scores_out = a->score_state_out ? 1 : 0;
+  w.with_state = with_state || a->state_in || a->score_state_in;
+  if (dev_out) {
+    w.t_iter = trace->iter; w.t_changed = trace->changed_node; w.t_movetype = trace->movetype;
+    w.t_gll = trace->global_ll; w.t_add = trace->additions; w.t_del = trace->deletions;
+    w.t_fn = trace->fn; w.t_fp = trace->fp;
+  } else {
+    CU_TRY(buf.alloc(&w.t_iter, n)); CU_TRY(buf.alloc(&w.t_changed, n));
+    CU_TRY(buf.alloc(&w.t_movetype, n)); CU_TRY(buf.alloc(&w.t_gll, n));
+    CU_TRY(buf.alloc(&w.t_add, n)); CU_TRY(buf.alloc(&w.t_del, n));
+    CU_TRY(buf.alloc(&w.t_fn, n)); CU_TRY(buf.alloc(&w.t_fp, n));
+  }
+  if (mcap) {
+    if (dev_out) w.moves = a->moves;
+    else CU_TRY(buf.alloc(&w.moves, (size_t)nc * mcap * 4));
+  }
+  if (a->edge_freq) {
+    if (dev_out) w.edge_freq = a->edge_freq;
+    else CU_TRY(buf.alloc(&w.edge_freq, (size_t)(nc * P * P)));
+    CU_TRY(cudaMemsetAsync(w.edge_freq, 0, (size_t)(nc * P * P) * 4, c->stream));
+  }
+  if (a->npar_freq) {
+    if (dev_out) w.npar_freq = a->npar_freq;
+    else CU_TRY(buf.alloc(&w.npar_freq, (size_t)(nc * P * (MP + 1))));
+    CU_TRY(buf.alloc(&w.npar_since, (size_t)(nc * P)));
+    CU_TRY(cudaMemsetAsync(w.npar_freq, 0, (size_t)(nc * P * (MP + 1)) * 4, c->stream));
+  }
+  int* d_seeds = nullptr;
+  CU_TRY(buf.alloc(&d_seeds, seeds.size()));
+  CU_TRY(cudaMemcpyAsync(d_seeds, up.p + u_seeds, seeds.size() * sizeof(int), cudaMemcpyHostToDevice, c->stream));
+  ra.seeds = d_seeds;
+  if (rmt) {
     int* d_pos = nullptr;
     CU_TRY(buf.alloc(&ra.mt_states, mt.size() * (w.pipeline ? 2 : 1)));
     CU_TRY(buf.alloc(&d_pos, (size_t)nc));
-    CU_TRY(cudaMemcpyAsync(ra.mt_states, mt.data(), mt.size() * 4, cudaMemcpyHostToDevice, c->stream));
+    CU_TRY(cudaMemcpyAsync(ra.mt_states, up.p + u_mt, mt.size() * 4, cudaMemcpyHostToDevice, c->stream));
     if (w.pipeline)
-      CU_TRY(cudaMemcpyAsync(ra.mt_states + mt.size(), mt.data(), mt.size() * 4, cudaMemcpyHostToDevice, c->stream));
-    CU_TRY(cudaMemcpyAsync(d_pos, mt_pos.data(), (size_t)nc * 4, cudaMemcpyHostToDevice, c->stream));
+      CU_TRY(cudaMemcpyAsync(ra.mt_states + mt.size(), up.p + u_mt, mt.size() * 4, cudaMemcpyHostToDevice, c->stream));
+    CU_TRY(cudaMemcpyAsync(d_pos, up.p + u_pos, (size_t)nc * 4, cudaMemcpyHostToDevice, c->stream));
     ra.mt_pos = d_pos;
   }
-  if (a->rng_kind == BN_RNG_REPLAY) {
+  if (replay) {
     double* d_rep = nullptr;
     CU_TRY(buf.alloc(&d_rep, (size_t)nc * a->replay_len));
-    CU_TRY(cudaMemcpyAsync(d_rep, a->replay, (size_t)nc * a->replay_len * 8, cudaMemcpyHostToDevice, c->stream));
+    CU_TRY(cudaMemcpyAsync(d_rep, up.p + u_rep, (size_t)nc * a->replay_len * 8, cudaMemcpyHostToDevice, c->stream));
     ra.replay = d_rep;
     ra.replay_len = a->replay_len;
   }
@@ -891,26 +1024,54 @@
 
   ChainResult* d_res = nullptr;
   CU_TRY(buf.alloc(&d_res, (size_t)nc));
-  tm.lap("workspace + seeds");
+  tm.lap("workspace + inputs queued");
   cudaEvent_t ev0, ev1;
   cudaEventCreate(&ev0); cudaEventCreate(&ev1);
   cudaEventRecord(ev0, c->stream);
   const char* msg = launch_chains(p, w, ra, d_res, nc, c->stream);
   c->launches++;
   cudaEventRecord(ev1, c->stream);
-  cudaError_t e = cudaStreamSynchronize(c->stream);
+  cudaError_t e = cudaSuccess;
+  if (!msg) {
+    auto d2h = [&](size_t off, const void* src, size_t bytes) {
+      if (e == cudaSuccess) e = cudaMemcpyAsync(dn.p + off, src, bytes, cudaMemcpyDeviceToHost, c->stream);
+    };
+    d2h(o_res, d_res, sizeof(ChainResult) * nc);
+    const cudaMemcpyKind fin_kind = dev_out ? cudaMemcpyDeviceToDevice : cudaMemcpyDeviceToHost;
+    if (dev_out) {
+      if (final_parents && e == cudaSuccess)
+        e = cudaMemcpyAsync(final_parents, w.par, (size_t)(nc * P * MP) * 4, fin_kind, c->stream);
+      if (final_n_par && e == cudaSuccess)
+        e = cudaMemcpyAsync(final_n_par, w.npar, (size_t)(nc * P) * 4, fin_kind, c->stream);
+    } else {
+      const void* cols[8] = {w.t_iter, w.t_changed, w.t_movetype, w.t_gll, w.t_add, w.t_del, w.t_fn, w.t_fp};
+      for (int k = 0; k < 8; k++) d2h(o_tr[k], cols[k], tr_bytes[k]);
+      if (mcap) d2h(o_mv, w.moves, (size_t)nc * mcap * 16);
+      if (a->edge_freq) d2h(o_ef, w.edge_freq, (size_t)(nc * P * P) * 4);
+      if (a->npar_freq) d2h(o_nf, w.npar_freq, (size_t)(nc * P * (MP + 1)) * 4);
+      if (final_parents) d2h(o_fp, w.par, (size_t)(nc * P * MP) * 4);
+      if (final_n_par) d2h(o_fn, w.npar, (size_t)(nc * P) * 4);
+    }
+    if (a->score_state_out && e == cudaSuccess) {
+      double* dst = dev_out ? a->score_state_out : dn.at<double>(o_sc);
+      e = cudaMemcpy2DAsync(dst, slen * 8, w.base, P * 8, P * 8, nc, fin_kind, c->stream);
+      if (MP > 8 && e == cudaSuccess)
+        e = cudaMemcpy2DAsync(dst + P, slen * 8, w.fac, (slen - P) * 8, (slen - P) * 8, nc, fin_kind, c->stream);
+    }
+  }
+  if (e == cudaSuccess) e = cudaStreamSynchronize(c->stream);
   if (e == cudaSuccess) e = cudaGetLastError();
   float ms = 0.f;
   if (e == cudaSuccess) cudaEventElapsedTime(&ms, ev0, ev1);
   cudaEventDestroy(ev0); cudaEventDestroy(ev1);
+  tm.lap("chain kernel + results D2H + sync");
+  int rc = ctx_settle(c);
+  if (rc) return rc;
   if (msg) return fail(BN_ERR_UNSUPPORTED, "%s", msg);
   if (e != cudaSuccess) return fail(BN_ERR_CUDA, "chain kernel: %s", cudaGetErrorString(e));
   if (kernel_ms) *kernel_ms = ms;
-  tm.lap("chain kernel + sync");
-
-  std::vector<ChainResult> res(nc);
-  CU_TRY(cudaMemcpy(res.data(), d_res, sizeof(ChainResult) * nc, cudaMemcpyDeviceToHost));
-  int rc = BN_OK;
+
+  const ChainResult* res = dn.at<ChainResult>(o_res);
   if (w.pipeline && getenv("BN_B200_PIPE_STATS"))
     for (int ch = 0; ch < nc && ch < 4; ch++)
       fprintf(stderr, "[bn_b200] chain %d two-CTA: %d windows requested, %d waits for the builder, %d discarded, %d in-place rebuilds, %lld cycles\n",
@@ -958,32 +1119,23 @@
       if (a->rng_kind == BN_RNG_WH) wh_advance(&seeds[3 * ch], res[ch].uniforms, o.wh_state);
     }
   }
-  if (a->score_state_out) {
-    const cudaMemcpyKind k = dev_out ? cudaMemcpyDeviceToDevice : cudaMemcpyDeviceToHost;
-    CU_TRY(cudaMemcpy2D(a->score_state_out, slen * 8, w.base, P * 8, P * 8, nc, k));
-    if (MP > 8) CU_TRY(cudaMemcpy2D(a->score_state_out + P, slen * 8, w.fac, (slen - P) * 8, (slen - P) * 8, nc, k));
-  }
-  const cudaMemcpyKind out_kind = dev_out ? cudaMemcpyHostToDevice : cudaMemcpyHostToHost;
-  CU_TRY(cudaMemcpy(trace->n_rows, nrows.data(), (size_t)nc * 4, out_kind));
-  if (a->n_moves) CU_TRY(cudaMemcpy(a->n_moves, nmoves.data(), (size_t)nc * 4, out_kind));
-  if (!dev_out) {
-    const size_t n = (size_t)(nc * cap);
-    CU_TRY(cudaMemcpy(trace->iter, w.t_iter, n * 4, cudaMemcpyDeviceToHost));
-    CU_TRY(cudaMemcpy(trace->changed_node, w.t_changed, n * 4, cudaMemcpyDeviceToHost));
-    CU_TRY(cudaMemcpy(trace->movetype, w.t_movetype, n * 4, cudaMemcpyDeviceToHost));
-    CU_TRY(cudaMemcpy(trace->global_ll, w.t_gll, n * 8, cudaMemcpyDeviceToHost));
-    CU_TRY(cudaMemcpy(trace->additions, w.t_add, n * 4, cudaMemcpyDeviceToHost));
-    CU_TRY(cudaMemcpy(trace->deletions, w.t_del, n * 4, cudaMemcpyDeviceToHost));
-    CU_TRY(cudaMemcpy(trace->fn, w.t_fn, n * 4, cudaMemcpyDeviceToHost));
-    CU_TRY(cudaMemcpy(trace->fp, w.t_fp, n * 4, cudaMemcpyDeviceToHost));
-    if (mcap) CU_TRY(cudaMemcpy(a->moves, w.moves, (size_t)nc * mcap * 16, cudaMemcpyDeviceToHost));
-    if (a->edge_freq) CU_TRY(cudaMemcpy(a->edge_freq, w.edge_freq, (size_t)(nc * P * P) * 4, cudaMemcpyDeviceToHost));
-    if (a->npar_freq) CU_TRY(cudaMemcpy(a->npar_freq, w.npar_freq, (size_t)(nc * P * (MP + 1)) * 4, cudaMemcpyDeviceToHost));
-  }
-  const cudaMemcpyKind fin_kind = dev_out ? cudaMemcpyDeviceToDevice : cudaMemcpyDeviceToHost;
-  if (final_parents) CU_TRY(cudaMemcpy(final_parents, w.par, (size_t)(nc * P * MP) * 4, fin_kind));
-  if (final_n_par) CU_TRY(cudaMemcpy(final_n_par, w.npar, (size_t)(nc * P) * 4, fin_kind));
-  tm.lap("results D2H");
+  if (dev_out) {
+    CU_TRY(cudaMemcpy(trace->n_rows, nrows.data(), (size_t)nc * 4, cudaMemcpyHostToDevice));
+    if (a->n_moves) CU_TRY(cudaMemcpy(a->n_moves, nmoves.data(), (size_t)nc * 4, cudaMemcpyHostToDevice));
+  } else {
+    memcpy(trace->n_rows, nrows.data(), (size_t)nc * 4);
+    if (a->n_moves) memcpy(a->n_moves, nmoves.data(), (size_t)nc * 4);
+    void* cols[8] = {trace->iter, trace->changed_node, trace->movetype, trace->global_ll, trace->additions,
+                     trace->deletions, trace->fn, trace->fp};
+    for (int k = 0; k < 8; k++) memcpy(cols[k], dn.p + o_tr[k], tr_bytes[k]);
+    if (mcap) memcpy(a->moves, dn.p + o_mv, (size_t)nc * mcap * 16);
+    if (a->edge_freq) memcpy(a->edge_freq, dn.p + o_ef, (size_t)(nc * P * P) * 4);
+    if (a->npar_freq) memcpy(a->npar_freq, dn.p + o_nf, (size_t)(nc * P * (MP + 1)) * 4);
+    if (final_parents) memcpy(final_parents, dn.p + o_fp, (size_t)(nc * P * MP) * 4);
+    if (final_n_par) memcpy(final_n_par, dn.p + o_fn, (size_t)(nc * P) * 4);
+    if (a->score_state_out) memcpy(a->score_state_out, dn.p + o_sc, (size_t)(nc * slen) * 8);
+  }
+  tm.lap("results unpacked");
   return rc;
 }
 
diff --git a/bayesnetworks_b200/csrc/gram.cu b/bayesnetworks_b200/csrc/gram.cu
--- a/bayesnetworks_b200/csrc/gram.cu
+++ b/bayesnetworks_b200/csrc/gram.cu
@@ -44,6 +44,7 @@
   mean[p] = acc / (double)n_samples;
 }
 
+constexpr int CENTER_PER_THREAD = 2;
 __global__ void __launch_bounds__(256) center_kernel(const double* X, int64_t ldx, int n_samples,
                                                      const double* __restrict__ mean, double* Xc,
                                                      int64_t ldc) {
@@ -51,8 +52,26 @@
   const double mu = mean[p];
   const double* src = X + (int64_t)p * ldx;
   double* dst = Xc + (int64_t)p * ldc;
-  for (int64_t n = (int64_t)blockIdx.x * 256 + threadIdx.x; n < ldc; n += (int64_t)gridDim.x * 256)
-    dst[n] = (n < n_samples) ? (src[n] - mu) : 0.0;
+  const bool vec = ((uintptr_t)src & 15) == 0;
+  for (int64_t n = CENTER_PER_THREAD * ((int64_t)blockIdx.x * 256 + threadIdx.x); n < ldc;
+       n += CENTER_PER_THREAD * (int64_t)gridDim.x * 256) {
+    double2 v;
+    if (vec && n + 1 < n_samples) {
+      const double2 x = *(const double2*)(src + n);
+      v.x = x.x - mu;
+      v.y = x.y - mu;
+    } else {
+      v.x = (n < n_samples) ? (src[n] - mu) : 0.0;
+      v.y = (n + 1 < n_samples) ? (src[n + 1] - mu) : 0.0;
+    }
+    *(double2*)(dst + n) = v;
+  }
+}
+
+static int center_blocks(int64_t ld_centered) {
+  const int64_t per_block = 256 * CENTER_PER_THREAD;
+  const int64_t gx = (ld_centered + per_block - 1) / per_block;
+  return gx > 1024 ? 1024 : (int)gx;
 }
 
 constexpr int TILE = 128;
@@ -296,14 +315,14 @@
 const char* gram_build(const double* dX, int64_t ldx, int n_samples, int P, double* dXc, int64_t ld_centered,
                        double* d_partial, const GramPlan& pl, double* d_colsum, double* d_mean,
                        double* d_C, int64_t ldc, double* d_scratch_part, int* d_error_flag,
-                       cudaStream_t stream, int64_t* launches, bool mean_given) {
+                       cudaStream_t stream, int64_t* launches, bool mean_given, cudaEvent_t x_read) {
   if (!mean_given) {
     gram_column_sums(dX, ldx, n_samples, P, d_scratch_part, d_colsum, d_mean, stream);
     if (launches) *launches += 2;
   }
-  int gx = (int)((ld_centered + 255) / 256);
-  if (gx > 1024) gx = 1024;
+  const int gx = center_blocks(ld_centered);
   center_kernel<<<dim3(gx, P), 256, 0, stream>>>(dX, ldx, n_samples, d_mean, dXc, ld_centered);
+  if (x_read) cudaEventRecord(x_read, stream);
   encode_fn_t enc = get_encode_fn();
   if (!enc) return "cuTensorMapEncodeTiled entry point not available";
   CUtensorMap tmap;
@@ -464,8 +483,7 @@
   int chunks = (int)((n_samples + 65535) / 65536);
   if (chunks < 1) chunks = 1;
   if (chunks > GRAM_MEAN_MAX_CHUNKS) chunks = GRAM_MEAN_MAX_CHUNKS;
-  int gx = (int)((ld_centered + 255) / 256);
-  if (gx > 1024) gx = 1024;
+  const int gx = center_blocks(ld_centered);
   StagePool& sp = StagePool::get();
   std::unique_lock<std::mutex> stage_lock(sp.use, std::defer_lock);
   bool staged = (size_t)n_samples * P * 8 >= ((size_t)32 << 20) && (size_t)n_samples * 8 <= STAGE_CHUNK &&
diff --git a/bayesnetworks_b200/csrc/gram.h b/bayesnetworks_b200/csrc/gram.h
--- a/bayesnetworks_b200/csrc/gram.h
+++ b/bayesnetworks_b200/csrc/gram.h
@@ -24,7 +24,8 @@
 const char* gram_build(const double* dX, int64_t ldx, int n_samples, int P, double* dXc,
                        int64_t ld_centered, double* d_partial, const GramPlan& pl, double* d_colsum,
                        double* d_mean, double* d_C, int64_t ldc, double* d_scratch_part,
-                       int* d_error_flag, cudaStream_t stream, int64_t* launches, bool mean_given = false);
+                       int* d_error_flag, cudaStream_t stream, int64_t* launches, bool mean_given = false,
+                       cudaEvent_t x_read = nullptr);
 
 const char* gram_build_from_host(const double* hX, int n_samples, int P, double* dXc, int64_t ld_centered,
                                  double* d_partial, const GramPlan& pl, double* d_colsum, double* d_mean,
```

Result: faster. 126.0 million (median of 6 runs) (+1.8%).
